# ishine/zerovox.cpp

Hardware: AMD Instinct MI355X
Metric: audio-seconds/wall-second (xRT) end-to-end phoneme->22.05 kHz wav (higher is better)
Workload: dtype f16*f16->f32 (MFMA) convs, f32 (MFMA) attention/linear, f32 activations

## Files before the change

zerovox.cpp_amd/csrc/capi.cpp:

```cpp
#include <algorithm>
#include <cmath>
#include <cstring>
#include <map>
#include <optional>
#include <string>
#include <thread>
#include <vector>

#include "common.h"
#include "model.h"
#include "knobs.h"

using zv::Model;

struct PendingBatch;
struct zv_model
{
    Model        *m;
    PendingBatch *pending;
};

static void free_pending(zv_model *m);
static void lane0_select(zv_model *m);
static void use_lane0(zv_model *m);
// ... 287 lines not shown
        const size_t b_ctl = r.prosody || tg ? zv::CTL_STRIDE * 4 : 0, b_pctl = pc ? (size_t)n * zv::PCTL_STRIDE * 4 : 0;
        if (!taps) M.reserve(n, T);
        Layout L;
        const size_t o_nf = L.at(4), o_ids = L.at(b_ids), o_pun = L.at(b_ids), o_sty = L.at(E * 4), o_ctl = L.at(b_ctl),
                     o_pctl = L.at(b_pctl), o_hid = L.at(b_hid);
        const size_t o_mel = taps ? 0 : L.at((size_t)T * M.hp.audio_num_mels * 4), o_wav = taps ? 0 : L.at(b_wav),
                     o_cum = taps ? 0 : L.at(dur ? b_ids : 0), o_live = L.at(r.fitted && !taps ? sizeof(zv::Seg) : 0),
                     o_runs = L.at(!r.fitted && !taps ? sizeof(zv::Seg) : 0);
        char *io = (char *)M.io_scratch(L.size());
        int32_t *d_nf = (int32_t *)(io + o_nf), *d_ids = (int32_t *)(io + o_ids), *d_pun = (int32_t *)(io + o_pun);
        float *d_sty = (float *)(io + o_sty), *d_hid = (float *)(io + o_hid);
        std::vector<float> ctl(b_ctl / 4), pctl(b_pctl / 4);
        std::vector<int32_t> cum(dur ? n : 0);
        pack_controls(r, ctl.data(), pctl.data());
        zv::Batch bt = zv::Batch::single(n, T, r.num_phonemes[0]);
        bt.has_targets = tg;
        if (r.fitted && !taps) bt.d_frm_live = (zv::Seg *)(io + o_live);
        if (!taps && M.dec_runs_on(bt)) bt.d_dec_runs = (zv::Seg *)(io + o_runs);
        ZV_HIP(hipMemcpyAsync(d_ids, r.ids[0], b_ids, hipMemcpyHostToDevice, M.stream()));
        ZV_HIP(hipMemcpyAsync(d_pun, r.puncts[0], b_ids, hipMemcpyHostToDevice, M.stream()));
        ZV_HIP(hipMemcpyAsync(d_sty, r.styles[0], E * 4, hipMemcpyHostToDevice, M.stream()));
        if (b_ctl)
        {
            bt.d_ctl = (const float *)(io + o_ctl);
            ZV_HIP(hipMemcpyAsync(io + o_ctl, ctl.data(), b_ctl, hipMemcpyHostToDevice, M.stream()));
        }
        if (b_pctl)
        {
            bt.d_pctl = (const float *)(io + o_pctl);
            ZV_HIP(hipMemcpyAsync(io + o_pctl, pctl.data(), b_pctl, hipMemcpyHostToDevice, M.stream()));
        }
        int32_t nf = 0;
        if (taps)
        {
            const Model::EncoderTaps t = M.encode_dev(bt, d_ids, d_pun, d_sty, d_hid, d_nf);
            ZV_HIP(hipMemcpyAsync(r.out[0], d_hid, b_hid, hipMemcpyDeviceToHost, M.stream()));
            ZV_HIP(hipMemcpyAsync(&nf, d_nf, 4, hipMemcpyDeviceToHost, M.stream()));
            if (taps->features) ZV_HIP(hipMemcpyAsync(taps->features, t.features, (size_t)n * E * 4, hipMemcpyDeviceToHost, M.stream()));
            if (taps->logdur) ZV_HIP(hipMemcpyAsync(taps->logdur, t.logdur, b_ids, hipMemcpyDeviceToHost, M.stream()));
            if (taps->pitch) ZV_HIP(hipMemcpyAsync(taps->pitch, t.pitch, b_ids, hipMemcpyDeviceToHost, M.stream()));
            if (taps->energy) ZV_HIP(hipMemcpyAsync(taps->energy, t.energy, b_ids, hipMemcpyDeviceToHost, M.stream()));
            if (taps->pitch_bucket) ZV_HIP(hipMemcpyAsync(taps->pitch_bucket, t.pitch_bucket, b_ids, hipMemcpyDeviceToHost, M.stream()));
            if (taps->energy_bucket) ZV_HIP(hipMemcpyAsync(taps->energy_bucket, t.energy_bucket, b_ids, hipMemcpyDeviceToHost, M.stream()));
            if (dur) ZV_HIP(hipMemcpyAsync(cum.data(), t.cum, b_ids, hipMemcpyDeviceToHost, M.stream()));
        }
        else
        {
            float *d_mel = (float *)(io + o_mel), *d_wav = (float *)(io + o_wav);
            if (dur) bt.d_cum = (int32_t *)(io + o_cum);
            M.chain_dev(bt, d_ids, d_pun, d_sty, d_hid, d_mel, d_wav, d_nf);
            ZV_HIP(hipMemcpyAsync(&nf, d_nf, 4, hipMemcpyDeviceToHost, M.stream()));
            if (dur) ZV_HIP(hipMemcpyAsync(cum.data(), bt.d_cum, b_ids, hipMemcpyDeviceToHost, M.stream()));
            ZV_HIP(hipMemcpyAsync(r.out[0], d_wav, b_wav, hipMemcpyDeviceToHost, M.stream()));
        }
        M.sync();
        if (r.n_frames) r.n_frames[0] = (uint32_t)nf;
        if (dur) durations_from_cum(cum.data(), 1, r.n, r.T, r.durations);
    });
}

zv_status zv_encode_taps(zv_model *m, const int32_t *ids, const int32_t *puncts, const float *style, uint32_t n,
                         uint32_t num_phonemes, uint32_t T, float *hidden, uint32_t *n_frames, float *features, float *logdur,
                         float *pitch, float *energy, int32_t *pitch_bucket, int32_t *energy_bucket)
{
    return run_single(m, {__func__, 1, &ids, &puncts, &style, &n, &num_phonemes, &T, &hidden, n_frames},
                      Taps{features, logdur, pitch, energy, pitch_bucket, energy_bucket});
}

zv_status zv_encode_taps_prosody(zv_model *m, const int32_t *ids, const int32_t *puncts, const float *style, uint32_t n,
                                 uint32_t num_phonemes, uint32_t T, float *hidden, uint32_t *n_frames, float *features, float *logdur,
                                 float *pitch, float *energy, int32_t *pitch_bucket, int32_t *energy_bucket, const zv_prosody *prosody)
{
    return run_single(m, {__func__, 1, &ids, &puncts, &style, &n, &num_phonemes, &T, &hidden, n_frames, prosody},
                      Taps{features, logdur, pitch, energy, pitch_bucket, energy_bucket});
}

zv_status zv_encode_taps_phonemes(zv_model *m, const int32_t *ids, const int32_t *puncts, const float *style, uint32_t n,
                                  uint32_t num_phonemes, uint32_t T, float *hidden, uint32_t *n_frames, float *features, float *logdur,
                                  float *pitch, float *energy, int32_t *pitch_bucket, int32_t *energy_bucket, const zv_prosody *prosody,
                                  const zv_phoneme_controls *phonemes, int32_t *durations)
{
    return run_single(m, {__func__, 1, &ids, &puncts, &style, &n, &num_phonemes, &T, &hidden, n_frames, prosody, phonemes, &durations},
                      Taps{features, logdur, pitch, energy, pitch_bucket, energy_bucket});
}

zv_status zv_encode(zv_model *m, const int32_t *ids, const int32_t *puncts, const float *style, uint32_t n, uint32_t T,
                    float *hidden, uint32_t *n_frames)
{
    return zv_encode_taps(m, ids, puncts, style, n, n, T, hidden, n_frames, nullptr, nullptr, nullptr, nullptr, nullptr, nullptr);
}

zv_status zv_decode(zv_model *m, const float *hidden, const float *style, uint32_t T, float *mel)
{
    return guarded([&] {
        ZV_NEED(m && hidden && style && mel, "null argument");
        Model &M = *m->m;
        use_lane0(m);
        check_T(M, T);
        const size_t E = M.E(), b_hid = (size_t)T * E * 4, b_mel = (size_t)T * M.hp.audio_num_mels * 4;
        Layout L;
        const size_t o_sty = L.at(E * 4), o_hid = L.at(b_hid), o_mel = L.at(b_mel);
        char *io = (char *)M.io_scratch(L.size());
        float *d_sty = (float *)(io + o_sty), *d_hid = (float *)(io + o_hid), *d_mel = (float *)(io + o_mel);
        ZV_HIP(hipMemcpyAsync(d_hid, hidden, b_hid, hipMemcpyHostToDevice, M.stream()));
        ZV_HIP(hipMemcpyAsync(d_sty, style, E * 4, hipMemcpyHostToDevice, M.stream()));
        M.decode_dev(zv::Batch::single(1, T, 1), d_hid, d_sty, d_mel);
        ZV_HIP(hipMemcpyAsync(mel, d_mel, b_mel, hipMemcpyDeviceToHost, M.stream()));
        M.sync();
    });
}

zv_status zv_vocode(zv_model *m, const float *mel, uint32_t T, float *wav)
{
    return guarded([&] {
        ZV_NEED(m && mel && wav, "null argument");
        Model &M = *m->m;
        use_lane0(m);
        check_T(M, T);
        const size_t b_mel = (size_t)T * M.hp.audio_num_mels * 4, b_wav = (size_t)T * M.hp.audio_hop_size * 4;
        Layout L;
        const size_t o_mel = L.at(b_mel), o_wav = L.at(b_wav);
        char *io = (char *)M.io_scratch(L.size());
        float *d_mel = (float *)(io + o_mel), *d_wav = (float *)(io + o_wav);
        ZV_HIP(hipMemcpyAsync(d_mel, mel, b_mel, hipMemcpyHostToDevice, M.stream()));
        M.vocode_dev_graph(zv::Batch::single(1, T, 1), d_mel, d_wav);
        ZV_HIP(hipMemcpyAsync(wav, d_wav, b_wav, hipMemcpyDeviceToHost, M.stream()));
        M.sync();
    });
}

uint32_t zv_vocoder_halo_frames(zv_model *m) { return m ? m->m->vocoder_halo_frames() : 0; }

zv_status zv_vocode_stream(zv_model *m, const float *mel, uint32_t T, uint32_t chunk_frames, zv_wav_sink sink, void *user)
{
    return guarded([&] {
        ZV_NEED(m && mel && sink, "null argument");
        ZV_NEED(T > 0 && chunk_frames > 0, "T and chunk_frames must be > 0");
        Model &M = *m->m;
        use_lane0(m);
        const size_t Mm = M.hp.audio_num_mels, hop = M.hp.audio_hop_size;
        const uint32_t H = M.vocoder_halo_frames();
        const uint32_t ctx_max = std::min<uint64_t>(T, (uint64_t)chunk_frames + 2 * H);
        check_T(M, ctx_max);
        struct RunsOff { Model &M; ~RunsOff() { M.voc_runs_off = false; } } runs_off{M};
        M.voc_runs_off = true;
        M.reserve(1, ctx_max);
        Layout L;
        const size_t o_mel = L.at((size_t)T * Mm * 4), o_wav = L.at((size_t)ctx_max * hop * 4);
        char *io = (char *)M.io_scratch(L.size());
        float *d_mel = (float *)(io + o_mel), *d_wav = (float *)(io + o_wav);
        Layout P;
        const size_t slot[2] = {P.at((size_t)chunk_frames * hop * 4), P.at((size_t)chunk_frames * hop * 4)};
        char *pin = (char *)M.pinned_scratch(P.size());
        hipEvent_t done[2] = {nullptr, nullptr};
        ZV_HIP(hipEventCreateWithFlags(&done[0], hipEventDisableTiming));
        ZV_HIP(hipEventCreateWithFlags(&done[1], hipEventDisableTiming));
        struct Pending { bool live; uint64_t first, n; } pend[2] = {{false, 0, 0}, {false, 0, 0}};
        auto deliver = [&](int k) {
            if (!pend[k].live) return;
            ZV_HIP(hipEventSynchronize(done[k]));
            sink(user, (const float *)(pin + slot[k]), pend[k].first, pend[k].n);
            pend[k].live = false;
        };
        try
        {
            ZV_HIP(hipMemcpyAsync(d_mel, mel, (size_t)T * Mm * 4, hipMemcpyHostToDevice, M.stream()));
            int k = 0;
            for (uint32_t a = 0; a < T; a += chunk_frames, k ^= 1)
            {
                const uint32_t b = std::min<uint64_t>(T, (uint64_t)a + chunk_frames);
                const uint32_t c0 = a > H ? a - H : 0, c1 = std::min<uint64_t>(T, (uint64_t)b + H);
                deliver(k);
                M.vocode_dev(zv::Batch::single(1, c1 - c0, 1), d_mel + (size_t)c0 * Mm, d_wav);
                ZV_HIP(hipMemcpyAsync(pin + slot[k], d_wav + (size_t)(a - c0) * hop, (size_t)(b - a) * hop * 4, hipMemcpyDeviceToHost, M.stream()));
                ZV_HIP(hipEventRecord(done[k], M.stream()));
                pend[k] = {true, (uint64_t)a * hop, (uint64_t)(b - a) * hop};
                deliver(k ^ 1);
            }
            deliver(k);
            deliver(k ^ 1);
        }
        catch (...)
        {
            hipStreamSynchronize(M.stream());
            hipEventDestroy(done[0]);
            hipEventDestroy(done[1]);
            throw;
        }
        M.sync();
        hipEventDestroy(done[0]);
        hipEventDestroy(done[1]);
    });
}

zv_status zv_synthesize(zv_model *m, const int32_t *ids, const int32_t *puncts, const float *style, uint32_t n, uint32_t T,
                        float *wav, uint32_t *n_frames)
{
    return run_single(m, {__func__, 1, &ids, &puncts, &style, &n, &n, &T, &wav, n_frames});
}

zv_status zv_synthesize_prosody(zv_model *m, const int32_t *ids, const int32_t *puncts, const float *style, uint32_t n, uint32_t T,
                                float *wav, uint32_t *n_frames, const zv_prosody *prosody)
{
    return run_single(m, {__func__, 1, &ids, &puncts, &style, &n, &n, &T, &wav, n_frames, prosody});
}

zv_status zv_synthesize_phonemes(zv_model *m, const int32_t *ids, const int32_t *puncts, const float *style, uint32_t n, uint32_t T,
                                 float *wav, uint32_t *n_frames, const zv_prosody *prosody, const zv_phoneme_controls *phonemes,
                                 int32_t *durations)
{
    return run_single(m, {__func__, 1, &ids, &puncts, &style, &n, &n, &T, &wav, n_frames, prosody, phonemes, &durations});
}

static void scatter_out(const char *pin_wav, const size_t *off, float *const *wav, const uint32_t *T, size_t hop, uint32_t a, uint32_t b)
{
    size_t total = 0;
    for (uint32_t u = a; u < b; u++) total += (size_t)T[u] * hop * 4;
    const unsigned nth = total > ((size_t)1 << 20) ? 4u : 1u;
    auto work = [&](unsigned k) {
        for (uint32_t u = a + k; u < b; u += nth) memcpy(wav[u], pin_wav + off[u], (size_t)T[u] * hop * 4);
    };
    if (nth == 1)
    {
        work(0);
        return;
    }
    std::vector<std::thread> th;
    for (unsigned k = 1; k < nth; k++) th.emplace_back(work, k);
    work(0);
    for (auto &t : th) t.join();
}

struct PendingBatch
{
    bool                  active = false;
    uint32_t              n_utt = 0;
    int                   G = 1;
    std::vector<uint32_t> gb;
    std::vector<size_t>   woff;
    std::vector<uint32_t> T;
    std::vector<float *>  wav;
    uint32_t             *n_frames = nullptr;
    const char           *h_wav = nullptr;
    const int32_t        *h_nf = nullptr;
    size_t                hop = 0;
    std::vector<uint32_t> N;
    std::vector<int32_t *> dur;
    const int32_t        *h_cum = nullptr;
};
static PendingBatch &pending_slot(zv_model *m, int lane)
{
    if (!m->pending) m->pending = new PendingBatch[ZV_BATCH_LANES];
    return m->pending[lane];
}
static void free_pending(zv_model *m)
{
    delete[] m->pending;
    m->pending = nullptr;
}
static void lane0_select(zv_model *m)
{
    if (hipSetDevice(m->m->device) != hipSuccess) zv::fail(ZV_ERR_DEVICE, "hipSetDevice(%d) failed", m->m->device);
    m->m->select_lane(0);
}
static void use_lane0(zv_model *m)
{
    if (m->pending && m->pending[0].active)
        zv::fail(ZV_ERR_ARG, "lane 0 has a batch in flight (zv_synthesize_batch_begin): finish it with zv_synthesize_batch_end first");
    if (hipSetDevice(m->m->device) != hipSuccess) zv::fail(ZV_ERR_DEVICE, "hipSetDevice(%d) failed", m->m->device);
    m->m->select_lane(0);
}

static void batch_enqueue(zv_model *m, int lane, const Request &r)
{
    Model &M = *m->m;
    PendingBatch &pb = pending_slot(m, lane);
    if (pb.active) zv::fail(ZV_ERR_ARG, "lane %d already has a batch in flight", lane);
    M.select_lane(lane);
    const size_t E = M.E(), Mm = M.hp.audio_num_mels, hop = M.hp.audio_hop_size;
    const bool tg = r.targets(), pc = r.phoneme_controls() || tg, ctl = r.prosody || tg, dur = r.timings();
    uint32_t nmax = 0, tmax = 0, ntot = 0;
    for (uint32_t u = 0; u < r.count; u++)
    {
        nmax = std::max(nmax, r.n[u]);
        tmax = std::max(tmax, r.T[u]);
        ntot += r.n[u];
    }
    zv::Batch bt;
    bt.nseg = (int)r.count;
    bt.n_max = zv::round_up((int)nmax, 32);
    bt.n_real = (int)nmax;
    bt.t_max = zv::round_up((int)tmax, 64);
    bt.n_rows = (size_t)bt.nseg * bt.n_max;
    bt.t_rows = (size_t)bt.nseg * bt.t_max;
    Layout in;
    const size_t b_tab = (size_t)(bt.nseg + 1) * sizeof(zv::Seg);
    const size_t i_tok = in.at(b_tab), i_frm = in.at(b_tab), i_ids = in.at(bt.n_rows * 4), i_pun = in.at(bt.n_rows * 4),
                 i_sty = in.at((size_t)bt.nseg * E * 4), i_ctl = in.at(ctl ? (size_t)bt.nseg * zv::CTL_STRIDE * 4 : 0),
                 i_pctl = in.at(pc ? bt.n_rows * zv::PCTL_STRIDE * 4 : 0), b_in = in.size();
    Layout dev;
    const size_t o_nf = dev.at((size_t)bt.nseg * 4), o_in = dev.at(b_in), o_hid = dev.at(bt.t_rows * E * 4),
                 o_mel = dev.at(bt.t_rows * Mm * 4), o_wav = dev.at(bt.t_rows * hop * 4), o_cum = dev.at(dur ? bt.n_rows * 4 : 0),
                 o_live = dev.at(r.fitted ? (size_t)bt.nseg * sizeof(zv::Seg) : 0),
                 o_runs = dev.at(!r.fitted ? (size_t)bt.nseg * sizeof(zv::Seg) : 0);
    M.reserve_batch(bt);
    char *io = (char *)M.io_scratch(dev.size());
    size_t wav_bytes = 0;
    pb.woff.assign(r.count, 0);
    for (uint32_t u = 0; u < r.count; u++)
    {
        pb.woff[u] = wav_bytes;
        wav_bytes += (size_t)r.T[u] * hop * 4;
    }
    Layout host;
    const size_t p_in = host.at(b_in), p_nf = host.at((size_t)bt.nseg * 4), p_wav = host.at(wav_bytes),
                 p_cum = host.at(dur ? bt.n_rows * 4 : 0);
    char *pin = (char *)M.pinned_scratch(host.size());
    char *d_in = io + o_in, *h_in = pin + p_in;
    {
        zv::Seg *h_tok = (zv::Seg *)(h_in + i_tok), *h_frm = (zv::Seg *)(h_in + i_frm);
        int32_t *h_ids = (int32_t *)(h_in + i_ids), *h_pun = (int32_t *)(h_in + i_pun);
        float *h_sty = (float *)(h_in + i_sty);
        int32_t n0 = 0, t0 = 0;
        for (uint32_t u = 0; u < r.count; u++)
        {
            const int32_t n = (int32_t)r.n[u], t = (int32_t)r.T[u];
            h_tok[u] = zv::Seg{n0, n, n, 0};
            h_frm[u] = zv::Seg{t0, t, 0, 0};
            memcpy(h_ids + n0, r.ids[u], (size_t)n * 4);
            memcpy(h_pun + n0, r.puncts[u], (size_t)n * 4);
            memcpy(h_sty + (size_t)u * E, r.styles[u], E * 4);
            n0 += n;
            t0 += t;
        }
        h_tok[r.count] = zv::Seg{0, n0, n0, 0};
        h_frm[r.count] = zv::Seg{0, t0, 0, 0};
        pack_controls(r, (float *)(h_in + i_ctl), (float *)(h_in + i_pctl));
    }
    bt.d_tok = (const zv::Seg *)(d_in + i_tok);
    bt.d_frm = (const zv::Seg *)(d_in + i_frm);
    if (ctl) bt.d_ctl = (const float *)(d_in + i_ctl);
    bt.has_targets = tg;
    if (pc) bt.d_pctl = (const float *)(d_in + i_pctl);
    if (dur) bt.d_cum = (int32_t *)(io + o_cum);
    if (r.fitted) bt.d_frm_live = (zv::Seg *)(io + o_live);
    if (M.dec_runs_on(bt)) bt.d_dec_runs = (zv::Seg *)(io + o_runs);
    int32_t *d_nf = (int32_t *)(io + o_nf), *d_ids = (int32_t *)(d_in + i_ids), *d_pun = (int32_t *)(d_in + i_pun);
    float *d_sty = (float *)(d_in + i_sty), *d_hid = (float *)(io + o_hid), *d_mel = (float *)(io + o_mel), *d_wav = (float *)(io + o_wav);
    int32_t *h_nf = (int32_t *)(pin + p_nf), *h_cum = dur ? (int32_t *)(pin + p_cum) : nullptr;
    char *h_wav = pin + p_wav;
    const int G = zv::voc_tail_groups(zv::knob(zv::ZV_TAIL_GROUPS), bt.nseg, wav_bytes, M.profiling, M.dbg_layer.kind >= 0);
    try
    {
        hipStream_t cs = M.copy_stream();
        pb.gb.assign(G + 1, r.count);
        pb.gb[0] = 0;
        const uint64_t seq = M.next_batch_seq();
        ZV_HIP(hipEventRecord(M.batch_event(seq, 0), M.stream()));
        if (G <= 1)
        {
            M.chain_dev(bt, d_ids, d_pun, d_sty, d_hid, d_mel, d_wav, d_nf, h_in, d_in, b_in);
            ZV_HIP(hipEventRecord(M.batch_event(seq, 1), M.stream()));
            ZV_HIP(hipMemcpyAsync(h_nf, d_nf, (size_t)bt.nseg * 4, hipMemcpyDeviceToHost, M.stream()));
            if (dur) ZV_HIP(hipMemcpyAsync(h_cum, bt.d_cum, (size_t)ntot * 4, hipMemcpyDeviceToHost, M.stream()));
            ZV_HIP(hipMemcpyAsync(h_wav, d_wav, wav_bytes, hipMemcpyDeviceToHost, M.stream()));
            ZV_HIP(hipEventRecord(M.tail_event(1), M.stream()));
        }
        else
        {
            M.chain_dev(bt, d_ids, d_pun, d_sty, d_hid, d_mel, d_wav, d_nf, h_in, d_in, b_in, 1);
            ZV_HIP(hipMemcpyAsync(h_nf, d_nf, (size_t)bt.nseg * 4, hipMemcpyDeviceToHost, M.stream()));
            if (dur) ZV_HIP(hipMemcpyAsync(h_cum, bt.d_cum, (size_t)ntot * 4, hipMemcpyDeviceToHost, M.stream()));
            for (int g = 1; g < G; g++)
            {
                uint32_t u = pb.gb[g - 1] + 1;
                while (u < r.count && pb.woff[u] < wav_bytes * g / G) u++;
                pb.gb[g] = std::min(u, r.count - (uint32_t)(G - g));
            }
            for (int g = 0; g < G; g++)
            {
                const uint32_t u0 = pb.gb[g], u1 = pb.gb[g + 1];
                M.vocode_tail(bt, d_mel, d_wav, (int)u0, (int)(u1 - u0));
                const size_t o0 = pb.woff[u0], o1 = u1 < r.count ? pb.woff[u1] : wav_bytes;
                ZV_HIP(hipEventRecord(M.tail_event(2 * g), M.stream()));
                ZV_HIP(hipStreamWaitEvent(cs, M.tail_event(2 * g), 0));
                ZV_HIP(hipMemcpyAsync(h_wav + o0, (const char *)d_wav + o0, o1 - o0, hipMemcpyDeviceToHost, cs));
                ZV_HIP(hipEventRecord(M.tail_event(2 * g + 1), cs));
            }
            ZV_HIP(hipEventRecord(M.batch_event(seq, 1), M.stream()));
        }
    }
    catch (...)
    {
        hipStreamSynchronize(M.stream());
        if (M.copy_stream()) hipStreamSynchronize(M.copy_stream());
        throw;
    }
    pb.active = true;
    pb.n_utt = r.count;
    pb.G = G;
    pb.T.assign(r.T, r.T + r.count);
    pb.wav.assign(r.out, r.out + r.count);
    pb.n_frames = r.n_frames;
    pb.h_wav = h_wav;
    pb.h_nf = h_nf;
    pb.hop = hop;
    pb.h_cum = h_cum;
    pb.N.assign(r.n, r.n + r.count);
    if (dur) pb.dur.assign(r.durations, r.durations + r.count);
    else pb.dur.clear();
}

static void batch_finish(zv_model *m, int lane)
{
    Model &M = *m->m;
    PendingBatch &pb = pending_slot(m, lane);
    if (!pb.active) zv::fail(ZV_ERR_ARG, "lane %d has no batch in flight", lane);
    M.select_lane(lane);
    try
    {
        for (int g = 0; g < pb.G; g++)
        {
            ZV_HIP(hipEventSynchronize(M.tail_event(2 * g + 1)));
            scatter_out(pb.h_wav, pb.woff.data(), pb.wav.data(), pb.T.data(), pb.hop, pb.gb[g], pb.gb[g + 1]);
        }
        M.sync();
    }
    catch (...)
    {
        hipStreamSynchronize(M.stream());
        if (M.copy_stream()) hipStreamSynchronize(M.copy_stream());
        pb.active = false;
        throw;
    }
    pb.active = false;
    if (pb.n_frames)
        for (uint32_t u = 0; u < pb.n_utt; u++) pb.n_frames[u] = (uint32_t)pb.h_nf[u];
    if (pb.h_cum) durations_from_cum(pb.h_cum, pb.n_utt, pb.N.data(), pb.T.data(), pb.dur.data());
}

static uint32_t batch_group_end(uint32_t a, uint32_t n_utt, const uint32_t *T)
{
    uint32_t b = a, tmax = 0;
    while (b < n_utt && b - a < 64)
    {
        const uint32_t tm = std::max(tmax, T[b]);
        if (b > a && (uint64_t)(b - a + 1) * zv::round_up((int)tm, 64) > 65536) break;
        tmax = tm;
        b++;
    }
    return b;
}

static zv_status synthesize_batch(zv_model *m, const Request &r)
{
      return guarded([&] {
        check_request(m, r);
        ZV_HIP(hipSetDevice(m->m->device));
        for (uint32_t a = 0, b; a < r.count; a = b)
        {
            b = batch_group_end(a, r.count, r.T);
            batch_enqueue(m, 0, r.slice(a, b));
            batch_finish(m, 0);
        }
    });
}

static zv_status begin_batch(zv_model *m, uint32_t lane, const Request &r)
{
    return guarded([&] {
        check_request(m, r);
        if (!(lane < ZV_BATCH_LANES)) zv::fail(ZV_ERR_ARG, "%s: lane out of range", r.fn);
        if (!(r.count > 0)) zv::fail(ZV_ERR_ARG, "%s: empty batch", r.fn);
        if (batch_group_end(0, r.count, r.T) != r.count)
            zv::fail(ZV_ERR_ARG, "%s: an asynchronous batch must fit one launch group (64 utterances, 64 Ki frames of capacity)", r.fn);
        ZV_HIP(hipSetDevice(m->m->device));
        batch_enqueue(m, (int)lane, r);
    });
}

zv_status zv_synthesize_batch(zv_model *m, uint32_t n_utt, const int32_t *const *ids, const int32_t *const *puncts,
                              const float *const *styles, const uint32_t *n_phonemes, const uint32_t *T, float *const *wav,
                              uint32_t *n_frames)
{
    return synthesize_batch(m, {__func__, n_utt, ids, puncts, styles, n_phonemes, n_phonemes, T, wav, n_frames});
}

zv_status zv_synthesize_batch_prosody(zv_model *m, uint32_t n_utt, const int32_t *const *ids, const int32_t *const *puncts,
                                      const float *const *styles, const uint32_t *n_phonemes, const uint32_t *T, float *const *wav,
                                      uint32_t *n_frames, const zv_prosody *prosody)
{
    return synthesize_batch(m, {__func__, n_utt, ids, puncts, styles, n_phonemes, n_phonemes, T, wav, n_frames, prosody});
}

zv_status zv_synthesize_batch_phonemes(zv_model *m, uint32_t n_utt, const int32_t *const *ids, const int32_t *const *puncts,
                                       const float *const *styles, const uint32_t *n_phonemes, const uint32_t *T, float *const *wav,
                                       uint32_t *n_frames, const zv_prosody *prosody, const zv_phoneme_controls *phonemes,
                                       int32_t *const *durations)
{
    return synthesize_batch(m, {__func__, n_utt, ids, puncts, styles, n_phonemes, n_phonemes, T, wav, n_frames, prosody, phonemes,
                                durations});
}

zv_status zv_synthesize_batch_begin(zv_model *m, uint32_t lane, uint32_t n_utt, const int32_t *const *ids, const int32_t *const *puncts,
                                    const float *const *styles, const uint32_t *n_phonemes, const uint32_t *T, float *const *wav,
                                    uint32_t *n_frames)
{
    return begin_batch(m, lane, {__func__, n_utt, ids, puncts, styles, n_phonemes, n_phonemes, T, wav, n_frames});
}

zv_status zv_synthesize_batch_begin_prosody(zv_model *m, uint32_t lane, uint32_t n_utt, const int32_t *const *ids,
                                            const int32_t *const *puncts, const float *const *styles, const uint32_t *n_phonemes,
                                            const uint32_t *T, float *const *wav, uint32_t *n_frames, const zv_prosody *prosody)
{
    return begin_batch(m, lane, {__func__, n_utt, ids, puncts, styles, n_phonemes, n_phonemes, T, wav, n_frames, prosody});
}

zv_status zv_synthesize_batch_begin_phonemes(zv_model *m, uint32_t lane, uint32_t n_utt, const int32_t *const *ids,
                                             const int32_t *const *puncts, const float *const *styles, const uint32_t *n_phonemes,
                                             const uint32_t *T, float *const *wav, uint32_t *n_frames, const zv_prosody *prosody,
                                             const zv_phoneme_controls *phonemes, int32_t *const *durations)
{
    return begin_batch(m, lane, {__func__, n_utt, ids, puncts, styles, n_phonemes, n_phonemes, T, wav, n_frames, prosody, phonemes,
                                 durations});
}

zv_status zv_synthesize_fitted(zv_model *m, const int32_t *ids, const int32_t *puncts, const float *style, uint32_t n, uint32_t T,
                               float *wav, uint32_t *n_frames, const zv_prosody *prosody, const zv_phoneme_controls *phonemes,
                               int32_t *durations)
{
    return run_single(m, {__func__, 1, &ids, &puncts, &style, &n, &n, &T, &wav, n_frames, prosody, phonemes, &durations, true});
}

zv_status zv_synthesize_batch_fitted(zv_model *m, uint32_t n_utt, const int32_t *const *ids, const int32_t *const *puncts,
                                     const float *const *styles, const uint32_t *n_phonemes, const uint32_t *T, float *const *wav,
                                     uint32_t *n_frames, const zv_prosody *prosody, const zv_phoneme_controls *phonemes,
                                     int32_t *const *durations)
{
    return synthesize_batch(m, {__func__, n_utt, ids, puncts, styles, n_phonemes, n_phonemes, T, wav, n_frames, prosody, phonemes,
                                durations, true});
}

zv_status zv_synthesize_batch_begin_fitted(zv_model *m, uint32_t lane, uint32_t n_utt, const int32_t *const *ids,
                                           const int32_t *const *puncts, const float *const *styles, const uint32_t *n_phonemes,
                                           const uint32_t *T, float *const *wav, uint32_t *n_frames, const zv_prosody *prosody,
                                           const zv_phoneme_controls *phonemes, int32_t *const *durations)
{
    return begin_batch(m, lane, {__func__, n_utt, ids, puncts, styles, n_phonemes, n_phonemes, T, wav, n_frames, prosody, phonemes,
                                 durations, true});
}

zv_status zv_encode_taps_target(zv_model *m, const int32_t *ids, const int32_t *puncts, const float *style, uint32_t n,
                                uint32_t num_phonemes, uint32_t T, float *hidden, uint32_t *n_frames, float *features, float *logdur,
                                float *pitch, float *energy, int32_t *pitch_bucket, int32_t *energy_bucket, const zv_prosody *prosody,
                                const zv_phoneme_controls *phonemes, int32_t *durations, uint32_t target_frames)
{
    return run_single(m, {__func__, 1, &ids, &puncts, &style, &n, &num_phonemes, &T, &hidden, n_frames, prosody, phonemes, &durations,
                          false, &target_frames},
                      Taps{features, logdur, pitch, energy, pitch_bucket, energy_bucket});
}

zv_status zv_synthesize_target(zv_model *m, const int32_t *ids, const int32_t *puncts, const float *style, uint32_t n, uint32_t T,
                               float *wav, uint32_t *n_frames, const zv_prosody *prosody, const zv_phoneme_controls *phonemes,
                               int32_t *durations, uint32_t target_frames, int fitted)
{
    return run_single(m, {__func__, 1, &ids, &puncts, &style, &n, &n, &T, &wav, n_frames, prosody, phonemes, &durations, fitted != 0,
                          &target_frames});
}

zv_status zv_synthesize_batch_target(zv_model *m, uint32_t n_utt, const int32_t *const *ids, const int32_t *const *puncts,
                                     const float *const *styles, const uint32_t *n_phonemes, const uint32_t *T, float *const *wav,
                                     uint32_t *n_frames, const zv_prosody *prosody, const zv_phoneme_controls *phonemes,
                                     int32_t *const *durations, const uint32_t *target_frames, int fitted)
{
    return synthesize_batch(m, {__func__, n_utt, ids, puncts, styles, n_phonemes, n_phonemes, T, wav, n_frames, prosody, phonemes,
                                durations, fitted != 0, target_frames});
}

zv_status zv_synthesize_batch_begin_target(zv_model *m, uint32_t lane, uint32_t n_utt, const int32_t *const *ids,
                                           const int32_t *const *puncts, const float *const *styles, const uint32_t *n_phonemes,
                                           const uint32_t *T, float *const *wav, uint32_t *n_frames, const zv_prosody *prosody,
                                           const zv_phoneme_controls *phonemes, int32_t *const *durations,
                                           const uint32_t *target_frames, int fitted)
{
    return begin_batch(m, lane, {__func__, n_utt, ids, puncts, styles, n_phonemes, n_phonemes, T, wav, n_frames, prosody, phonemes,
                                 durations, fitted != 0, target_frames});
}

zv_status zv_synthesize_batch_end(zv_model *m, uint32_t lane)
{
    return guarded([&] {
        ZV_NEED(m, "null argument");
        ZV_NEED(lane < ZV_BATCH_LANES, "lane out of range");
        ZV_HIP(hipSetDevice(m->m->device));
        batch_finish(m, (int)lane);
    });
}

zv_status zv_batch_timeline(zv_model *m, uint32_t cap, double *start_ms, double *end_ms, uint32_t *n)
{
    return guarded([&] {
        ZV_NEED(m && start_ms && end_ms && n, "null argument");
        Model &M = *m->m;
        ZV_HIP(hipSetDevice(M.device));
        M.sync_all_lanes();
        const uint64_t total = M.batch_seq();
        const uint64_t cnt = std::min<uint64_t>(std::min<uint64_t>(cap, total), (uint64_t)Model::BATCH_RING);
// ... 358 lines not shown
```

zerovox.cpp_amd/csrc/conv_plan.h:

```cpp
#pragma once

#include <stddef.h>

#include "conv_xcd.h"
#include "knobs.h"
#include "tile_deal.h"

namespace zv
{

constexpr long BATCH_ROWS = 16384;
inline bool batch_switch(int value, bool picked_by_itself) { return value != 0 && (value == 2 || picked_by_itself); }
inline bool batch_rows(long rows) { return rows >= BATCH_ROWS; }

constexpr size_t LDS_PER_WG = 160 * 1024;
constexpr size_t LDS_TWO_WGS = 80 * 1024;
constexpr size_t LDS_DEFAULT = 64 * 1024;

inline int plan_round_up(int x, int a) { return (x + a - 1) / a * a; }

struct ConvCall
{
    int njobs, nseg, max_rows, rate, n_cu, nt_begin;
};

inline int conv_gemm_groups(int Cout_p) { return ((Cout_p + 31) / 32) / 8; }
inline int conv_gemm_tiles(int Cout_p)
{
    const int nt = (Cout_p + 31) / 32, ng = nt / 8;
    return ng * 8 + ((nt - ng * 8 == 1 && ng >= 1) ? 1 : 0);
}
inline int conv_gemm_units(int Cin_p, int K)
{
    int n = 0;
    for (int c0 = 0; c0 < Cin_p; c0 += 256) n += K * (((Cin_p - c0 < 256 ? Cin_p - c0 : 256) + 63) / 64);
    return n;
}

enum ConvPrologue : int
{
    PRO_RAW_F16 = 0,
    PRO_ACT = 1,
    PRO_NORM_ACT = 2,
    PRO_MELNORM = 3,
    PRO_SUM3_ACT = 4,
    PRO_SCALE_ACT = 5
};

#ifndef ZV_SINGLE_LW
#define ZV_SINGLE_LW 4
#endif
#ifndef ZV_CONV_BATCH_ROUTE
#define ZV_CONV_BATCH_ROUTE 1
#endif

struct ConvDesc
{
    int  K, dil, pad, Cin_p, Cout_p, ck, pro, ldx;
    bool has_w8, out_f16, has_res, has_stat, eact, three_inputs;
};

inline bool conv_gemm_takes(const ConvDesc &j, const ConvCall &c)
{
    const long rows = (long)c.max_rows * c.rate * c.nseg;
    return batch_switch(knob(ZV_CONV_GEMM), batch_rows(rows)) && j.has_w8 && j.pro == PRO_RAW_F16 && j.Cin_p >= 128 &&
           conv_gemm_groups(j.Cout_p) >= 1 && !j.out_f16 && (j.ldx & 7) == 0;
}

struct ConvGemmPlan
{
    int    order, tps, gx, threads;
    size_t lds_bytes;
};
inline ConvGemmPlan conv_gemm_plan(int Cout_p, const ConvCall &c)
{
    ConvGemmPlan p{};
    p.order = knob(ZV_GEMM_ORDER);
    p.tps = (c.max_rows * c.rate + 255) / 256;
    const int ng = conv_gemm_groups(Cout_p), rts = p.tps * c.nseg;
    p.gx = (p.order == 1 && (ng == 1 || ng == 2 || ng == 4)) ? plan_round_up(rts, 8 / ng) * ng : rts * ng;
    p.threads = 512;
    p.lds_bytes = 4 * (16384 + 18432);
    return p;
}

inline bool conv_stream_ok(const ConvDesc &j, const ConvCall &c)
{
    return c.njobs == 1 && c.nt_begin == 0 && (j.pro == PRO_ACT || j.pro == PRO_SCALE_ACT) && j.K == 3 && j.dil == 1 && j.pad == 1 &&
           (j.Cin_p == 64 || j.Cin_p == 128) && j.ck == j.Cin_p && (j.ldx & 3) == 0 && !j.has_res && !j.has_stat && !j.eact && !j.out_f16 &&
           !j.three_inputs;
}

inline bool conv_tiled_exists(int MT, int WN, int NT)
{
    return (NT == 1 && (MT == 1 || MT == 2 || MT == 4) && (WN == 1 || WN == 2 || WN == 4)) || (NT == 2 && MT == 2 && WN == 4);
}

enum ConvForm { CONV_STREAM, CONV_LOADER, CONV_TILED };
struct ConvPlan
{
    bool     valid;
    ConvForm form;
    int      MT, WN, NT;
    int      strip, nkc;
    int      tps;
    int      gx, gy, gz, threads;
    size_t   lds_bytes;
    int      tile_bytes;
    int      xcd_nx, xcd_ny, xcd_spread;
    int      warm;
};

inline bool conv_plan_tiles(ConvPlan &p, bool loader, int MT, int WN, int NT, int Lmax, int ntiles, int halo, int ck, int dmax, const ConvCall &c)
{
    const int BM = 32 * MT * (4 / WN);
    p.form = loader ? CONV_LOADER : CONV_TILED;
    p.MT = MT, p.WN = WN, p.NT = NT;
    p.tps = (Lmax + BM - 1) / BM;
    p.gx = p.tps * c.nseg, p.gy = (ntiles + WN * NT - 1) / (WN * NT), p.gz = c.njobs;
    const int LW = loader ? ZV_SINGLE_LW : 0;
    p.threads = 256 + 64 * LW;
    p.xcd_nx = p.xcd_ny = p.xcd_spread = 0;
    p.warm = knob(ZV_CONV_WARM) != 0;
    if (loader && knob(ZV_CONV_XCD) != 0)
    {
        p.xcd_ny = p.gy;
        p.xcd_nx = p.gx;
        p.xcd_spread = c.nseg > 1;
        p.gx = conv_xcd_grid(p.xcd_nx, p.xcd_ny, p.xcd_spread), p.gy = 1;
    }
    p.tile_bytes = plan_round_up((BM + halo + dmax) * (ck * 2 + 16), 16);
    p.lds_bytes = (size_t)p.tile_bytes * (LW > 0 ? 2 : 1);
    return p.lds_bytes <= LDS_PER_WG;
}

inline ConvPlan conv_stream_plan(const ConvDesc &j, const ConvCall &c)
{
    ConvPlan p{};
    const int Lmax = c.max_rows * c.rate;
    const int ntiles = (j.Cout_p + 31) / 32, gy = (ntiles + 3) / 4;
    const int occ = j.Cin_p == 128 ? 2 : 3;
    int strip = 8;
    while (strip > 2 && (long)((Lmax + 64 * strip - 1) / (64 * strip)) * c.nseg * gy < 12L * occ * c.n_cu) strip >>= 1;
    p.valid = true;
    p.form = CONV_STREAM;
    p.strip = strip;
    p.nkc = j.Cin_p / 16;
    p.tps = (Lmax + 64 * strip - 1) / (64 * strip);
    p.gx = p.tps * c.nseg, p.gy = gy, p.gz = 1;
    p.threads = 256;
    p.lds_bytes = (size_t)2 * 66 * (j.Cin_p * 2 + 16);
    return p;
}

inline ConvPlan conv_plan(const ConvDesc *jobs, const ConvCall &c)
{
    ConvPlan p{};
    const int njobs = c.njobs, n_cu = c.n_cu;
    const int Lmax = c.max_rows * c.rate;
    if (njobs < 1) return p;
    int halo = 0, ck = 0, dmax = 1;
    for (int i = 0; i < njobs; i++)
    {
        dmax = jobs[i].dil > dmax ? jobs[i].dil : dmax;
        if (jobs[i].Cout_p != jobs[0].Cout_p) return p;
        const int h = (jobs[i].K - 1) * jobs[i].dil;
        if (h > halo) halo = h;
        ck = jobs[i].ck > ck ? jobs[i].ck : ck;
    }
    const int Cout_p = jobs[0].Cout_p;
    const int ntiles = (Cout_p + 31) / 32 - c.nt_begin;
    if (ntiles < 1) return p;
    const int WN = ntiles >= 3 ? 4 : (ntiles >= 2 ? 2 : 1);
    auto wgs = [&](int MT, int NT) {
        const int BM = 32 * MT * (4 / WN);
        return (long)((Lmax + BM - 1) / BM) * c.nseg * ((ntiles + WN * NT - 1) / (WN * NT)) * njobs;
    };
    int MT = 4;
    while (MT > 1 && wgs(MT, 1) < 2L * n_cu) MT >>= 1;
    while (MT > 1 && (size_t)(32 * MT * (4 / WN) + halo + dmax) * (ck * 2 + 16) > LDS_TWO_WGS) MT >>= 1;
    {
        const double ai = 2.0 * jobs[0].K * jobs[0].Cin_p * Cout_p / (4.0 * (jobs[0].Cin_p + Cout_p));
        const bool memory_bound = ai < 200.0 && wgs(1, 1) >= 16L * n_cu;
        if (conv_stream_ok(jobs[0], c) && batch_switch(knob(ZV_CONV_STREAM), memory_bound)) return conv_stream_plan(jobs[0], c);
        if (memory_bound && MT > 2) MT = 2;
    }
    if (MT < knob(ZV_CONV_MT)) MT = knob(ZV_CONV_MT);
    const int nt_env = knob(ZV_CONV_NT);
    int NT = (WN == 4 && ntiles >= 8 && MT >= 2 && wgs(MT, 2) >= 4L * n_cu && jobs[0].K * jobs[0].Cin_p >= 2048) ? 2 : 1;
    if (nt_env == 1 || (nt_env == 2 && WN == 4 && ntiles >= 2 && MT >= 2)) NT = nt_env;
    if (NT == 2 && MT == 4) MT = 2;
    {
        const bool batch_rounds = ZV_CONV_BATCH_ROUTE && c.nseg > 1 && wgs(1, 1) > n_cu;
        const int  single_env = knob(ZV_CONV_SINGLE);
        if (single_env != 0 && MT == 1 && NT == 1 && ck == 256 && wgs(1, 1) <= 2L * n_cu && !batch_rounds && (jobs[0].Cin_p > 256 || single_env == 2) &&
            WN >= 2 && conv_plan_tiles(p, true, 1, WN, 1, Lmax, ntiles, halo, ck, dmax, c))
        {
            p.valid = true;
            return p;
        }
    }
    p.valid = conv_tiled_exists(MT, WN, NT) && conv_plan_tiles(p, false, MT, WN, NT, Lmax, ntiles, halo, ck, dmax, c);
    return p;
}

constexpr int TRIPLE_MAX_DIL = 3;

struct BlockTile
{
    int sumd, dmax;
    int h2;
    int halo;
    int TM;
};
inline BlockTile block_tile(int K, const int *dil, int n_dil, int R)
{
    BlockTile t{0, 1, (K - 1) / 2, 0, 0};
    for (int d = 0; d < n_dil; d++)
    {
        t.sumd += dil[d];
        t.dmax = dil[d] > t.dmax ? dil[d] : t.dmax;
    }
    t.halo = t.h2 * (t.sumd + n_dil);
    t.TM = R - 2 * t.halo;
    return t;
}

struct BlockDesc
{
    int Cp, K, n_dil;
    int dil[TRIPLE_MAX_DIL];
};

inline bool pair_supported(int Cp, int K)
{
    if (!(Cp == 32 || Cp == 64 || Cp == 128 || Cp == 256) || K < 1 || (K & 1) == 0) return false;
    const int nsb = (K * (Cp / 16) + 3) >> 2;
    return nsb >= 2 && (Cp == 64 || (nsb & 1) == 0);
}
inline bool triple_supported(int Cp, int K, const int *dil, int n_dil)
{
    if (Cp != 32 || n_dil < 1 || n_dil > TRIPLE_MAX_DIL || !pair_supported(Cp, K) || (K & 1) == 0) return false;
    return block_tile(K, dil, n_dil, 256).TM >= 96;
}
inline bool block64_supported(int Cp, int K, const int *dil, int n_dil)
{
    if (Cp != 64 || K < 3 || (K & 1) == 0 || n_dil < 1 || n_dil > TRIPLE_MAX_DIL) return false;
    return block_tile(K, dil, n_dil, 256).TM >= 192;
}

struct PairPlan
{
    bool   valid;
    bool   ring;
    int    MT;
    int    deal_c, gx, gz;
    int    ring_off;
    size_t lds_bytes;
};
inline PairPlan pair_plan(int Cp, int Kmax, int dmax, bool any_sum, bool merged, bool all_ring_weights, const ConvCall &c)
{
    PairPlan p{};
    if (!(Cp == 32 || Cp == 64 || Cp == 128 || Cp == 256) || (any_sum && merged)) return p;
    const int  njobs = c.njobs, n_cu = c.n_cu, Lmax = c.max_rows * c.rate;
    const int  WN = Cp == 256 ? 4 : Cp / 32;
    auto wgs = [&](int MT) {
        const int BM = 32 * MT * (4 / WN);
        const int TM = BM - (Kmax - 1);
        return TM < 32 ? 0L : (long)((Lmax + TM - 1) / TM) * c.nseg * njobs;
    };
    p.deal_c = tile_deal_chunk(Cp);
    p.gz = merged ? 1 : njobs;
    {
        const int  ring_env = knob(ZV_PAIR64_RING);
        const bool ok = Cp == 64 && !any_sum && ring_env != 0 && Kmax >= 3 &&
                        (size_t)(256 + Kmax * dmax) * 144 + 4 * 8192 + 1024 <= LDS_TWO_WGS && all_ring_weights;
        const long rwgs = (long)((Lmax + 256 - Kmax) / (257 - Kmax)) * c.nseg * njobs;
        if (ok && (ring_env == 2 || rwgs >= 6L * n_cu))
        {
            const int BM = 256, TMmin = BM - (Kmax - 1);
            p.ring = true;
            p.gx = tile_deal_grid((Lmax + TMmin - 1) / TMmin, c.nseg, p.deal_c);
            p.ring_off = plan_round_up((BM + Kmax * dmax) * (64 * 2 + 16), 1024);
            p.lds_bytes = (size_t)p.ring_off + 4 * 8192;
            p.valid = p.lds_bytes <= LDS_TWO_WGS;
            return p;
        }
    }
    int MT = (Cp == 128 && wgs(4) >= 8L * n_cu) ? 4 : 2;
    if (Cp == 256 && !merged && wgs(3) >= 4L * n_cu) MT = 3;
    const int mt_env = knob(ZV_PAIR_MT);
    if (mt_env == 2 || mt_env == 4 || (mt_env == 3 && Cp == 256 && !merged)) MT = mt_env;
    p.MT = MT;
    const int BM = 32 * MT * (4 / WN);
    const int TMmin = BM - (Kmax - 1);
    if (TMmin < 32) return p;
    p.gx = tile_deal_grid((Lmax + TMmin - 1) / TMmin, c.nseg, p.deal_c);
    p.lds_bytes = (size_t)(BM + (Kmax + (Cp == 256 ? 0 : (Cp >= 128 ? 1 : 4))) * dmax) * (Cp * 2 + 16);
    p.valid = true;
    return p;
}

struct TriplePlan
{
    bool   valid;
    int    R, MT;
    bool   lds_form;
    int    db_mask;
    int    interleave;
    int    deal_c, gx, gz, threads;
    size_t lds_bytes;
};
inline TriplePlan triple_plan(const BlockDesc *jobs, const ConvCall &c)
{
    TriplePlan p{};
    const int njobs = c.njobs, Lmax = c.max_rows * c.rate;
    const int v2_env = knob(ZV_TRIPLE_V2);
    const int R = ((long)Lmax * c.nseg * njobs >= 7000L * c.n_cu || v2_env == 3) ? 512 : 256;
    p.R = R, p.MT = 2;
    p.deal_c = tile_deal_chunk(32);
    p.interleave = 1;
    int    gx = 8;
    size_t lds = 0, lds2 = 0;
    for (int i = 0; i < njobs; i++)
    {
        const BlockDesc &P = jobs[i];
        if (P.Cp != jobs[0].Cp || !triple_supported(P.Cp, P.K, P.dil, P.n_dil)) return p;
        const BlockTile t = block_tile(P.K, P.dil, P.n_dil, R);
        const int g = tile_deal_grid((Lmax + t.TM - 1) / t.TM, c.nseg, p.deal_c);
        gx = g > gx ? g : gx;
        const size_t rows = R + 2 * t.h2 * t.dmax + 5 * t.dmax;
        const size_t b = rows * (P.Cp * 2 + 16);
        lds = b > lds ? b : lds;
        const int    nb = ((P.K * 2 + 3) >> 2) >> 1;
        const size_t one = (size_t)plan_round_up((int)(rows * 80), 1024) + (size_t)(8 * nb + 2) * 1024 + 1024;
        const bool   db = knob(ZV_TRIPLE_DB) != 0 && one + (size_t)8 * nb * 1024 <= LDS_TWO_WGS;
        if (db) p.db_mask |= 1 << i;
        const size_t b2 = one + (db ? (size_t)8 * nb * 1024 : 0);
        lds2 = b2 > lds2 ? b2 : lds2;
    }
    if (njobs < 1 || lds > LDS_DEFAULT) return p;
    p.gx = gx, p.gz = njobs;
    if (v2_env && (R == 512 || v2_env >= 2) && lds2 <= LDS_TWO_WGS)
    {
        p.lds_form = true;
        p.interleave = knob(ZV_TRIPLE_INTERLEAVE) != 0 ? njobs : 1;
        if (p.interleave > 1) p.gx = gx * njobs, p.gz = 1;
        p.threads = R;
        p.lds_bytes = lds2;
        p.valid = true;
        return p;
    }
    p.db_mask = 0;
    p.threads = 64 * (R / 32 / p.MT);
    p.lds_bytes = lds;
    p.valid = true;
    return p;
}

struct Block64Plan
{
    bool   valid;
    int    deal_c, gx, gz, threads;
    int    ring_off;
    size_t lds_bytes;
};
inline Block64Plan block64_plan(const BlockDesc *jobs, const ConvCall &c)
{
    Block64Plan p{};
    const int Lmax = c.max_rows * c.rate;
    p.deal_c = tile_deal_chunk(64);
    int gx = 8, rows_max = 0;
    for (int i = 0; i < c.njobs; i++)
    {
        const BlockDesc &P = jobs[i];
        if (!block64_supported(P.Cp, P.K, P.dil, P.n_dil)) return p;
        const BlockTile t = block_tile(P.K, P.dil, P.n_dil, 256);
        const int g = tile_deal_grid((Lmax + t.TM - 1) / t.TM, c.nseg, p.deal_c);
        gx = g > gx ? g : gx;
        const int rows = 256 + 2 * t.h2 * t.dmax + 2 * t.dmax;
        rows_max = rows > rows_max ? rows : rows_max;
    }
    p.gx = gx, p.gz = c.njobs, p.threads = 256;
    p.ring_off = plan_round_up(rows_max * (64 * 2 + 16), 1024);
    p.lds_bytes = (size_t)p.ring_off + 4 * 8192;
    p.valid = c.njobs >= 1 && p.lds_bytes <= LDS_TWO_WGS;
    return p;
}

}
```

zerovox.cpp_amd/csrc/dec_runs.h:

```cpp
#pragma once

#include <stddef.h>

#if defined(__HIPCC__)
#define ZV_DR_FN __host__ __device__ static inline
#else
#define ZV_DR_FN static inline
#endif

namespace zv
{

constexpr int DEC_RUN_BLOCK = 32;
constexpr int DEC_RUN_MARGIN = 32;

struct DecRun
{
    int rows_c;
    int gap_at;
    int G;
};

ZV_DR_FN DecRun dec_run(int n, int T, int R)
{
    const DecRun whole = {T, 0, 0};
    n = n < 0 ? 0 : (n < T ? n : T);
    if (R < 0 || T - R - 1 < 0) return whole;
    const long a = ((long)n + R + 2 * DEC_RUN_BLOCK - 1) / DEC_RUN_BLOCK * DEC_RUN_BLOCK;
    const long b = (long)(T - R - 1) / DEC_RUN_BLOCK * DEC_RUN_BLOCK;
    if (b - a < DEC_RUN_BLOCK || b - a < DEC_RUN_MARGIN) return whole;
    const DecRun r = {(int)(a + (T - b)), (int)(a / DEC_RUN_BLOCK), (int)((b - a) / DEC_RUN_BLOCK)};
    return r;
}

ZV_DR_FN int dec_run_compact_row(int t, int gap_at, int G)
{
    const int a = gap_at * DEC_RUN_BLOCK, b = a + G * DEC_RUN_BLOCK;
    return (G <= 0 || t < a) ? t : (t < b ? a - 1 : t - G * DEC_RUN_BLOCK);
}
ZV_DR_FN int dec_run_original_row(int c, int gap_at, int G) { return (G <= 0 || c < gap_at * DEC_RUN_BLOCK) ? c : c + G * DEC_RUN_BLOCK; }

ZV_DR_FN void dec_run_block_sum(const double *p, size_t stride, int nb, int gap_at, int G, double *sum, double *sumsq)
{
    double s1 = 0.0, s2 = 0.0;
    for (int b0 = 0; b0 < nb; b0 += 8)
    {
        double v1[8], v2[8];
#if defined(__HIPCC__)
#pragma unroll
#endif
        for (int i = 0; i < 8; i++)
        {
            const double *q = p + (size_t)(b0 + i < nb ? b0 + i : nb - 1) * stride;
            v1[i] = q[0];
            v2[i] = q[1];
        }
#if defined(__HIPCC__)
#pragma unroll
#endif
        for (int i = 0; i < 8; i++)
            if (b0 + i < nb)
            {
                s1 += v1[i];
                s2 += v2[i];
                if (b0 + i + 1 == gap_at)
                    for (int k = 0; k < G; k++)
                    {
                        s1 += v1[i];
                        s2 += v2[i];
                    }
            }
    }
    *sum = s1;
    *sumsq = s2;
}

}
```

zerovox.cpp_amd/csrc/decoder.cpp:

```cpp
#include "schedule.h"

#include <algorithm>
#include <cmath>

namespace zv
{

Model::DecLayout Model::dec_layout(DeviceArena &a, const Batch &bt) const
{
    const size_t S = (size_t)bt.nseg, L = bt.t_rows, B = 2 * E(), R = (size_t)dec_.R, CAT = B + R;
    DecLayout d{(bt.t_max + 31) / 32, round_up(dec_.fc_out + 64, 64), 2 * (int)CAT + 64};
    d.h = a.take_n<float>(S * d.hs);
    for (float **st : {&d.st_x, &d.st_t, &d.st_y, &d.st_a}) *st = a.take_n<float>(S * d.ss);
    for (double **p : {&d.part_t, &d.part_o}) *p = a.take_n<double>(S * d.nblk * CAT * 2);
    d.cat = a.take_n<float>(L * CAT);
    for (float **x : {&d.t1, &d.sc, &d.x0, &d.xa}) *x = a.take_n<float>(L * B);
    d.asr_t = a.take_n<float>(L * R);
    d.xa16 = a.take_n<_Float16>(L * CAT);
    d.t16 = a.take_n<_Float16>(L * B);
    d.xr16 = a.take_n<_Float16>(L * CAT);
    d.mel_c = a.take_n<float>(L * dec_.M);
    return d;
}

bool Model::dec_prepass_on(const Batch &bt) const
{
    const int pre_env = knob(ZV_DEC_PREPASS);
    return pre_env >= 0 ? pre_env != 0 : (size_t)bt.t_max * bt.nseg >= 256;
}

bool Model::dec_runs_on(const Batch &bt) const
{
    const int k = knob(ZV_DEC_RUNS);
    return !bt.d_frm_live && dbg_layer.kind < 0 && dec_prepass_on(bt) && batch_switch(k, batch_rows((long)bt.t_rows));
}

int Model::dec_reach_frames() const
{
    auto half = [](const ConvW &w) { return w.K > 0 ? (w.K - 1) / 2 : 0; };
    auto blk = [&](const DecBlk &b) { return std::max(half(b.conv1) + half(b.conv2), b.learned_sc ? half(b.sc) : 0); };
    int r = std::max(blk(dec_.enc[0]) + blk(dec_.enc[1]), half(dec_.asr0));
    for (const DecBlk &b : dec_.dec) r += blk(b);
    return r + half(dec_.to_out);
}

void Model::decode_dev(const Batch &bt, const float *d_hidden, const float *d_styles, float *d_mel)
{
    if (bt.t_rows == 0 || bt.t_max <= 0) fail(ZV_ERR_ARG, "T must be > 0");
    const DecLayout lay = dec_layout(stage_arena(bt), bt);
    const bool runs = bt.d_dec_runs != nullptr;
    if (runs && !dec_runs_on(bt)) fail(ZV_ERR_ARG, "internal: a decoder run table on a schedule that takes none");
    const Segs fr = runs ? Segs{bt.d_dec_runs, bt.nseg, bt.t_max, bt.frm1} : bt.frames();
    const int Ed = (int)E(), B = 2 * Ed, R = dec_.R, CAT = B + R, S = bt.nseg;
    const size_t L = bt.t_rows;
    const int nblk = lay.nblk, hs = lay.hs, ss = lay.ss;
    float *const h = lay.h, *const st_x = lay.st_x, *const st_t = lay.st_t, *const st_y = lay.st_y, *const st_a = lay.st_a;
    double *const part_t = lay.part_t, *const part_o = lay.part_o;
    float *const cat = lay.cat, *const t1 = lay.t1, *const sc = lay.sc, *const x0 = lay.x0, *const xa = lay.xa, *const asr_t = lay.asr_t;
    _Float16 *const xa16 = lay.xa16, *const t16 = lay.t16, *const xr16 = lay.xr16;
    double Ld = (double)L;
    if (runs && profiling)
    {
        std::vector<Seg> tab((size_t)S);
        ZV_HIP(hipMemcpyAsync(tab.data(), bt.d_dec_runs, tab.size() * sizeof(Seg), hipMemcpyDeviceToHost, stream()));
        ZV_HIP(hipStreamSynchronize(stream()));
        Ld = 0;
        for (const Seg &g : tab) Ld += g.rows;
    }
    const bool prepass = dec_prepass_on(bt);

    ZV_LAUNCH("dec_adain_fc", 4.0 * dec_.fc_out * (Ed + 2), 2.0 * S * dec_.fc_out * Ed,
              launch_linear(stream(), d_styles, Ed, Ed, dec_.fcW, dec_.fcB, dec_.fc_out, h, hs, dec_.fcExtra, segs_single(S)));

    const float rsqrt2 = (float)(1.0 / sqrt(2.0));

    auto finalize = [&](const double *part, int C, float *stat, int c_off) {
        ZV_LAUNCH("dec_in_stats", 16.0 * S * nblk * C, 4.0 * S * nblk * C,
                  launch_stats_finalize(stream(), part, nblk, C, 1e-5f, stat, ss, c_off, fr, 1, runs));
    };
    auto norm_input = [&](ConvJob &j, const float *x, int ldx, int C, const double *part, int Cpart, float *stat, const float *g,
                          const float *b, int gb_seg, _Float16 *op16, _Float16 *raw16 = nullptr) {
        if (prepass)
        {
            ZV_LAUNCH("dec_norm_operand", 6.0 * Ld * C, 8.0 * Ld * C,
                      launch_norm_act_f16(stream(), x, ldx, C, part, nblk, Cpart, 1e-5f, stat, ss, g, b, gb_seg, 0.2f, op16, C, fr, raw16, runs));
            j.x0 = op16;
            j.ldx = C;
            j.pro = PRO_RAW_F16;
        }
        else
        {
            finalize(part, Cpart, stat, 0);
            j.x0 = x;
            j.ldx = ldx;
            j.pro = PRO_NORM_ACT;
            j.pstat = stat;
            j.pstat_seg = ss;
            j.pa = g;
            j.pb = b;
            j.pab_seg = gb_seg;
            j.slope = 0.2f;
        }
    };

    ZV_LAUNCH("dec_in_stats", 4.0 * Ld * Ed, 3.0 * Ld * Ed, launch_stats_partial(stream(), d_hidden, Ed, Ed, part_o, nblk, fr, 1));

    int blk_no = 0;
    auto block = [&](const DecBlk &b, const float *x, int ldx, int Cpart, float *st_in, const float *g1, const float *b1,
                     const float *g2, const float *b2, int gb_seg, float *out, int ldo, bool want_stats) {
        const bool dbg_here = dbg_layer.kind == 2 && dbg_layer.index == blk_no && !dbg_layer.done;
        blk_no++;
        if (dbg_layer.done) return;
        if (dbg_here)
        {
            dbg_inject(const_cast<float *>(x), ldx, b.cin, L);
            ZV_HIP(launch_stats_partial(stream(), x, ldx, b.cin, part_o, nblk, fr, 1));
            Cpart = b.cin;
        }
        const float *res = x;
        int ldres = ldx;
        ConvJob jj[2];
        int nj = 0;
        {
            ConvJob j = job(b.conv1);
            norm_input(j, x, ldx, b.cin, part_o, Cpart, st_in, g1, b1, gb_seg, xa16, b.learned_sc ? xr16 : nullptr);
            j.out = t1;
            j.stat_part = part_t;
            j.stat_nblk = nblk;
            j.stat_C = b.conv1.Cout;
            jj[nj++] = j;
        }
        double bytes = conv_bytes(Ld, b.cin, b.conv1.Cout, 3, false), flops = conv_flops(Ld, b.cin, b.conv1.Cout, 3);
        if (b.learned_sc)
        {
            ConvJob j = job(b.sc);
            j.x0 = x;
            j.ldx = ldx;
            if (prepass)
            {
                j.x0 = xr16;
                j.ldx = b.cin;
                j.pro = PRO_RAW_F16;
            }
            j.out = sc;
            res = sc;
            ldres = b.sc.Cout_p;
            const double sb = conv_bytes(Ld, b.cin, b.cout, 1, false), sf = conv_flops(Ld, b.cin, b.cout, 1);
            if (b.sc.Cout_p == b.conv1.Cout_p)
            {
                jj[nj++] = j;
                bytes += sb;
                flops += sf;
            }
            else
                conv(&j, 1, fr, 1, "dec_conv", sb, sf);
        }
        conv(jj, nj, fr, 1, "dec_conv", bytes, flops);
        const int Cm = b.conv1.Cout;
        {
            ConvJob j = job(b.conv2);
            norm_input(j, t1, b.conv1.Cout_p, Cm, part_t, Cm, st_t, g2, b2, gb_seg, t16);
            j.res = res;
            j.ldres = ldres;
            j.escale = rsqrt2;
            j.out = out;
            j.ldo = ldo;
            if (want_stats)
            {
                j.stat_part = part_o;
                j.stat_nblk = nblk;
                j.stat_C = b.cout;
            }
            conv(&j, 1, fr, 1, "dec_conv", conv_bytes(Ld, Cm, b.cout, 3, true), conv_flops(Ld, Cm, b.cout, 3));
        }
        if (dbg_here) dbg_extract(out, ldo, b.cout, L);
    };

    if (dbg_layer.kind == ZV_LAYER_DEC_ADAIN)
    {
        const int bi = dbg_layer.index / 2, k = dbg_layer.index & 1;
        if (bi < 0 || bi >= 5) return;
        const DecBlk &b = dec_.dec[bi];
        const int Cn = k ? b.cout : b.cin, go = k ? b.g2 : b.g1;
        float *xin = cat;
        dbg_inject(xin, Cn, Cn, L);
        ZV_HIP(launch_stats_partial(stream(), xin, Cn, Cn, part_o, nblk, fr, 1));
        ZV_HIP(launch_stats_finalize(stream(), part_o, nblk, Cn, 1e-5f, st_x, ss, 0, fr, 1));
        ZV_HIP(launch_norm_apply(stream(), xin, Cn, Cn, st_x, ss, h + go, h + go + Cn, t1, Cn, nullptr, nblk, fr));
        dbg_extract(t1, Cn, Cn, L);
        return;
    }

    block(dec_.enc[0], d_hidden, Ed, Ed, st_x, dec_.enc[0].n1w, dec_.enc[0].n1b, dec_.enc[0].n2w, dec_.enc[0].n2b, 0, x0, B, true);
    block(dec_.enc[1], x0, B, B, st_y, dec_.enc[1].n1w, dec_.enc[1].n1b, dec_.enc[1].n2w, dec_.enc[1].n2b, 0, cat, CAT, true);

    if (dbg_layer.done) return;
    {
        ConvJob j = job(dec_.asr0);
        j.x0 = d_hidden;
        j.ldx = Ed;
        j.out = asr_t;
        j.stat_part = part_t;
        j.stat_nblk = nblk;
        j.stat_C = R;
        conv(&j, 1, fr, 1, "dec_conv", conv_bytes(Ld, Ed, R, 1, false), conv_flops(Ld, Ed, R, 1));
        finalize(part_t, R, st_a, 0);
        ZV_LAUNCH("dec_norm_apply", 8.0 * Ld * R, 3.0 * Ld * R,
                  launch_norm_apply(stream(), asr_t, R, R, st_a, ss, dec_.asr1w, dec_.asr1b, cat + B, CAT, part_t, nblk, fr));
        finalize(part_t, R, st_x, B);
        if (dbg_layer.kind == ZV_LAYER_DEC_ASR_RES)
        {
            dbg_extract(cat + B, CAT, R, L);
            return;
        }
    }

    const float *cur = cat;
    int ldc = CAT;
    float *outs[5] = {cat, cat, xa, x0, xa};
    const int ldos[5] = {CAT, CAT, Ed, Ed, Ed};
    const int cparts[5] = {B, B, B, Ed, Ed};
    float *sts[5] = {st_x, st_x, st_x, st_y, st_y};
    for (int i = 0; i < 5; i++)
    {
        const DecBlk &b = dec_.dec[i];
        block(b, cur, ldc, cparts[i], sts[i], h + b.g1, h + b.g1 + b.cin, h + b.g2, h + b.g2 + b.cout, hs, outs[i], ldos[i], i < 4);
        cur = outs[i];
        ldc = ldos[i];
    }
    if (dbg_layer.done) return;
    {
        ConvJob j = job(dec_.to_out);
        j.x0 = cur;
        j.ldx = ldc;
        j.out = runs ? lay.mel_c : d_mel;
        j.ldo = dec_.M;
        if (dbg_layer.kind == ZV_LAYER_DEC_TO_OUT) dbg_inject(const_cast<float *>(cur), ldc, Ed, L);
        conv(&j, 1, fr, 1, "dec_conv", conv_bytes(Ld, Ed, dec_.M, 1, false), conv_flops(Ld, Ed, dec_.M, 1));
        if (dbg_layer.kind == ZV_LAYER_DEC_TO_OUT) dbg_extract(d_mel, dec_.M, dec_.M, L);
    }
    if (runs)
        ZV_LAUNCH("dec_run_expand", 4.0 * (Ld + (double)L) * dec_.M, 0.0,
                  launch_dec_run_expand(stream(), lay.mel_c, d_mel, dec_.M, fr, bt.frames_cap()));
}

}
```

zerovox.cpp_amd/csrc/encoder.cpp:

```cpp
#include "schedule.h"

#include <cmath>

namespace zv
{

Model::EncLayout Model::enc_layout(DeviceArena &a, const Batch &bt) const
{
    const size_t n = bt.n_rows, Ed = E();
    EncLayout e{round_up(enc_.dur.V, 16)};
    for (float **p : {&e.x, &e.y}) *p = a.take_n<float>(n * Ed);
    e.qkv = a.take_n<float>(n * 3 * Ed);
    for (float **p : {&e.o, &e.f}) *p = a.take_n<float>(n * Ed);
    e.hh = a.take_n<_Float16>(n * round_up(hp.conv_filter_size, 16));
    for (float **p : {&e.va, &e.vb}) *p = a.take_n<float>(n * e.Vp);
    for (float **p : {&e.t.logdur, &e.t.pitch, &e.t.energy}) *p = a.take_n<float>(n);
    for (int32_t **p : {&e.t.pitch_bucket, &e.t.energy_bucket}) *p = a.take_n<int32_t>(n);
    e.t.cum = bt.d_cum ? bt.d_cum : a.take_n<int32_t>(n);
    e.t.features = e.x;
    return e;
}

Model::EncoderTaps Model::encode_dev(const Batch &bt, const int32_t *d_ids, const int32_t *d_puncts, const float *d_styles,
                                     float *d_hidden, int32_t *d_nframes)
{
    if (bt.n_rows == 0 || bt.t_rows == 0 || bt.n_max <= 0 || bt.t_max <= 0) fail(ZV_ERR_ARG, "N and T must be > 0");
    const int n_longest = bt.n_real > 0 ? bt.n_real : bt.n_max;
    if (n_longest > enc_.posenc_rows) fail(ZV_ERR_ARG, "%d phonemes exceed the %d rows of the sinusoid table", n_longest, enc_.posenc_rows);
    const EncLayout lay = enc_layout(stage_arena(bt), bt);
    const Segs tk = bt.tokens(), fr = bt.frames_cap();
    const Segs tkm = knob(ZV_LINEAR_MERGED) != 0 ? bt.tokens_merged() : tk;
    const int Ed = (int)E(), H = hp.encoder_head, dk = Ed / H;
    const size_t n = bt.n_rows;
    const double nd = (double)n;
    const int Vp = lay.Vp;
    float *const x = lay.x, *const y = lay.y, *const qkv = lay.qkv, *const o = lay.o, *const f = lay.f, *const va = lay.va, *const vb = lay.vb;
    _Float16 *const hh = lay.hh;
    const bool tails = dbg_layer.kind < 0 && knob(ZV_LN_TAIL) != 0 && layernorm_tail_ok(Ed) && layernorm_tail_ok(enc_.dur.V);
    const EncoderTaps t = lay.t;

    ZV_LAUNCH("enc_embed", 8.0 * nd * Ed, 1.0 * nd * Ed,
              launch_embed(stream(), d_ids, d_puncts, enc_.wemb, hp.emb_dim, enc_.pemb, hp.punct_emb_dim, enc_.posenc, x, Ed, tk));
    if (dbg_layer.kind == ZV_LAYER_ENC_EMBED)
    {
        dbg_extract(x, Ed, Ed, n);
        return t;
    }
    const float temperature = (float)pow((double)dk, 0.5);
    const float inv_t = (float)(1.0 / temperature);
    int layer_no = 0;
    for (const EncLayer &Ly : enc_.layers)
    {
        const bool dbg_here = dbg_layer.kind == 1 && dbg_layer.index == layer_no;
        const bool dbg_mha = dbg_layer.kind == ZV_LAYER_ENC_MHA && dbg_layer.index == layer_no;
        const bool dbg_ffn = dbg_layer.kind == ZV_LAYER_ENC_FFN && dbg_layer.index == layer_no;
        layer_no++;
        if (dbg_here || dbg_mha) dbg_inject(x, Ed, Ed, n);
        ZV_LAUNCH("enc_linear", 4.0 * (3.0 * Ed * Ed + 4.0 * nd * Ed), 6.0 * nd * Ed * Ed,
                  launch_linear(stream(), x, Ed, Ed, Ly.qkvW, Ly.qkvB, 3 * Ed, qkv, 3 * Ed, nullptr, tkm));
        ZV_LAUNCH("enc_attention", 16.0 * nd * Ed, 4.0 * nd * bt.n_max * Ed,
                  launch_attention(stream(), qkv, qkv + Ed, qkv + 2 * Ed, 3 * Ed, H, dk, inv_t, o, Ed, tk));
        ZV_LAUNCH("enc_linear", 4.0 * (1.0 * Ed * Ed + 2.0 * nd * Ed), 2.0 * nd * Ed * Ed,
                  launch_linear(stream(), o, Ed, Ed, Ly.fcW, Ly.fcB, Ed, f, Ed, nullptr, tkm));
        ZV_LAUNCH("enc_layernorm", 12.0 * nd * Ed, 8.0 * nd * Ed,
                  launch_add_layernorm(stream(), f, Ed, x, Ed, Ed, Ed, Ly.ln1w, Ly.ln1b, 1e-5f, y, Ed, tkm));
        if (dbg_mha)
        {
            dbg_extract(y, Ed, Ed, n);
            return t;
        }
        if (dbg_ffn) dbg_inject(y, Ed, Ed, n);
        {
            ConvJob a = job(Ly.w1);
            a.x0 = y;
            a.eact = 1;
            a.oslope = 0.f;
            a.out_f16 = 1;
            a.out = hh;
            conv(&a, 1, tk, 1, "enc_conv", conv_bytes(nd, Ed, Ly.w1.Cout, Ly.w1.K, false), conv_flops(nd, Ed, Ly.w1.Cout, Ly.w1.K));
            ConvJob b = job(Ly.w2);
            b.x0 = hh;
            b.pro = PRO_RAW_F16;
            b.out = f;
            conv(&b, 1, Ly.w2.K == 1 ? tkm : tk, 1, "enc_conv", conv_bytes(nd, Ly.w1.Cout, Ed, Ly.w2.K, false), conv_flops(nd, Ly.w1.Cout, Ed, Ly.w2.K));
        }
        if (tails && layer_no == (int)enc_.layers.size())
            ZV_LAUNCH("enc_layernorm", 12.0 * nd * Ed, 9.0 * nd * Ed,
                      launch_layernorm_tail(stream(), f, Ed, y, Ed, Ed, Ed, Ly.ln2w, Ly.ln2b, 1e-5f, x, Ed, tk, d_styles, Ed, nullptr, nullptr,
                                            nullptr, nullptr, 0, 0, nullptr, 0, nullptr));
        else
            ZV_LAUNCH("enc_layernorm", 12.0 * nd * Ed, 8.0 * nd * Ed,
                      launch_add_layernorm(stream(), f, Ed, y, Ed, Ed, Ed, Ly.ln2w, Ly.ln2b, 1e-5f, x, Ed, tkm));
        if (dbg_here || dbg_ffn)
        {
            dbg_extract(x, Ed, Ed, n);
            return t;
        }
    }
    if (!(tails && !enc_.layers.empty()))
        ZV_LAUNCH("enc_add_style", 8.0 * nd * Ed, 1.0 * nd * Ed, launch_add_rowvec(stream(), x, Ed, Ed, d_styles, Ed, tk));

    int pred_no = 0;
    auto predictor = [&](const VarPred &v, float *out, const float *emb, int32_t *bucket, int ctl_field, int pctl_field) {
        const float *pctl = emb && bt.d_pctl ? bt.d_pctl + pctl_field : nullptr;
        const bool dbg_here = dbg_layer.kind == 3 && dbg_layer.index == pred_no && !dbg_layer.done;
        pred_no++;
        if (dbg_layer.done) return;
        if (dbg_here) dbg_inject(x, Ed, Ed, n);
        ConvJob a = job(v.c1);
        a.x0 = x;
        a.eact = 1;
        a.oslope = 0.f;
        a.out = va;
        conv(&a, 1, tk, 1, "enc_conv", conv_bytes(nd, Ed, v.V, 3, false), conv_flops(nd, Ed, v.V, 3));
        ZV_LAUNCH("enc_layernorm", 8.0 * nd * v.V, 8.0 * nd * v.V,
                  launch_add_layernorm(stream(), va, Vp, nullptr, 0, v.V, Vp, v.l1w, v.l1b, 1e-5f, vb, Vp, tkm));
        ConvJob b = job(v.c2);
        b.x0 = vb;
        b.pad = 1;
        b.eact = 1;
        b.oslope = 0.f;
        b.out = va;
        conv(&b, 1, tk, 1, "enc_conv", conv_bytes(nd, v.V, v.V, 3, false), conv_flops(nd, v.V, v.V, 3));
        if (tails)
        {
            ZV_LAUNCH("enc_layernorm", 8.0 * nd * v.V + (emb ? 12.0 * nd * Ed : 0.0), 10.0 * nd * v.V,
                      launch_layernorm_tail(stream(), va, Vp, nullptr, 0, v.V, Vp, v.l2w, v.l2b, 1e-5f, vb, Vp, tk, nullptr, 0, v.lw, v.lb, out,
                                            emb, (int)hp.encoder_ve_n_bins, Ed, x, Ed, bucket, emb ? bt.d_ctl : nullptr, ctl_field, pctl));
            return;
        }
        ZV_LAUNCH("enc_layernorm", 8.0 * nd * v.V, 8.0 * nd * v.V,
                  launch_add_layernorm(stream(), va, Vp, nullptr, 0, v.V, Vp, v.l2w, v.l2b, 1e-5f, vb, Vp, tkm));
        ZV_LAUNCH("enc_rowdot", 4.0 * nd * v.V, 2.0 * nd * v.V, launch_rowdot(stream(), vb, Vp, v.V, v.lw, v.lb, out, tk));
        if (dbg_here) dbg_extract(out, 1, 1, n);
        if (emb && !dbg_layer.done)
            ZV_LAUNCH("enc_bucket_embed", 12.0 * nd * Ed, 1.0 * nd * Ed,
                      launch_bucket_embed_add(stream(), out, hp.encoder_ve_n_bins, emb, Ed, x, Ed, bucket, tk, bt.d_ctl, ctl_field, pctl));
    };
    predictor(enc_.dur, t.logdur, nullptr, nullptr, 0, 0);
    predictor(enc_.pitch, t.pitch, enc_.pitch_emb, t.pitch_bucket, CTL_PITCH, PCTL_PITCH);
    if (dbg_layer.done) return t;
    predictor(enc_.energy, t.energy, enc_.energy_emb, t.energy_bucket, CTL_ENERGY, PCTL_ENERGY);
    if (dbg_layer.done) return t;
    if (bt.has_targets)
    {
        if (!bt.d_ctl || !bt.d_pctl) fail(ZV_ERR_ARG, "a batch with target durations needs its control rows");
        ZV_LAUNCH("enc_fit_durations", 24.0 * nd, 0.0, launch_fit_durations(stream(), t.logdur, bt.d_ctl, bt.d_pctl, tk, fr));
    }
    ZV_LAUNCH("enc_length_regulator", 4.0 * (nd + (double)bt.t_rows) * Ed, 0.0,
              launch_length_regulator(stream(), x, Ed, t.logdur, Ed, d_hidden, Ed, t.cum, d_nframes, tk, fr, bt.d_ctl, bt.d_pctl));
    if (bt.d_frm_live)
        ZV_LAUNCH("enc_live_frames", 36.0 * bt.nseg, 0.0, launch_live_frames(stream(), d_nframes, bt.d_frm_live, fr));
    if (bt.d_dec_runs)
        ZV_LAUNCH("enc_dec_runs", 36.0 * bt.nseg, 0.0, launch_dec_runs(stream(), d_nframes, bt.d_dec_runs, fr, dec_reach_frames()));
    return t;
}

void Model::debug_layernorm(int index, uint32_t n)
{
    const int l = index >> 1, Ed = (int)E();
    if (index < 0 || l >= (int)enc_.layers.size()) return;
    const EncLayer &Ly = enc_.layers[l];
    float *d = (float *)io_scratch(2 * (size_t)n * Ed * 4), *y = d + (size_t)n * Ed;
    dbg_inject(d, Ed, Ed, n);
    ZV_HIP(launch_add_layernorm(stream(), d, Ed, nullptr, 0, Ed, Ed, (index & 1) ? Ly.ln2w : Ly.ln1w, (index & 1) ? Ly.ln2b : Ly.ln1b,
                                1e-5f, y, Ed, segs_single((int)n)));
    dbg_extract(y, Ed, Ed, n);
}

}
```

zerovox.cpp_amd/csrc/kernels.h:

```cpp
#pragma once

#include <hip/hip_runtime.h>
#include <stdint.h>

#include "conv_plan.h"
#include "voc_plan.h"

#ifdef ZV_DIAG
#define ZV_DBGBITS(x) (x)
#else
#define ZV_DBGBITS(x) 0
#endif

namespace zv
{

__host__ __device__ static inline int round_up(int x, int a) { return (x + a - 1) / a * a; }

struct Seg
{
    int32_t row0, rows;
    int32_t aux;
    int32_t pad;
};
struct Segs
{
    const Seg *tab;
    int        nseg;
    int        max_rows;
    Seg        one;
};
__host__ __device__ static inline Seg seg_at(const Segs &s, int u)
{
    Seg g = s.tab ? s.tab[u] : s.one;
#if defined(__HIP_DEVICE_COMPILE__)
    g.row0 = __builtin_amdgcn_readfirstlane(g.row0);
    g.rows = __builtin_amdgcn_readfirstlane(g.rows);
    g.aux = __builtin_amdgcn_readfirstlane(g.aux);
#endif
    return g;
}
static inline Segs segs_single(int rows, int aux = 0)
{
    Segs s;
    s.tab = nullptr;
    s.nseg = 1;
    s.max_rows = rows;
    s.one.row0 = 0;
    s.one.rows = rows;
    s.one.aux = aux;
    s.one.pad = 0;
    return s;
}


struct ConvJob
{
    const void  *x0, *x1, *x2;
    int          ldx;
    int          pro;
    float        slope, pscale;
    const float *pa, *pb;
    const float *pstat;
    int          L, Cin_p, Cout_p, K, dil, pad;
    int          ck;
    const void  *w;
    const void  *w8;
    const float *bias;
    const float *res;
    int          ldres;
    float        escale;
    int          eact;
    float        oslope;
    int          out_f16;
    void        *out;
    int          ldo;
    int          dbg;
    int          pstat_seg, pab_seg;
    double      *stat_part;
    int          stat_nblk, stat_C;
};

constexpr int CONV_MAX_JOBS = 4;
struct ConvJobs
{
    ConvJob j[CONV_MAX_JOBS];
    Segs    segs;
    int     rate;
    int     tps;
    int     nt_begin;
    int     order;
    int     tile_bytes;
    int     xcd_ny, xcd_nx;
    int     xcd_spread;
    int     warm;
#ifdef ZV_STAMPS
    unsigned long long *stamp;
#endif
};

size_t packed_conv_weight_halfs(int Cin_p, int Cout_p, int K);
int    conv_pick_ck(int Cin_p, int ck_max = 0);
void   pack_conv_weight(const uint16_t *w, int K, int IC, int OC, int Cin_p, int Cout_p, int ck, uint16_t *dst);
size_t conv_gemm_weight_halfs(int Cin_p, int Cout_p, int K);
void   pack_conv_weight_gemm(const uint16_t *w, int K, int IC, int OC, int Cin_p, int Cout_p, uint16_t *dst);
hipError_t launch_conv(hipStream_t s, const ConvJob *jobs, int njobs, int n_cu, const Segs &segs, int rate);

struct PairJob
{
    const float *y;
    float       *out;
    const void  *w1, *w2;
    const void  *w1r, *w2r;
    const float *b1, *b2;
    int          L, Cp, K, dil;
    float        slope;
    int          dbg;
    const float *sum_in;
    float       *sum_out;
};
constexpr int PAIR_MAX_JOBS = 3;
struct PairJobs
{
    PairJob j[PAIR_MAX_JOBS];
    Segs    segs;
    int     rate;
    int     njobs, kmax;
    int     deal_c;
#ifdef ZV_STAMPS
    unsigned long long *stamp;
#endif
    float  *merge_out;
    int     ring_off;
};
size_t     pair_weight_halfs(int Cp, int K);
void       pack_pair_weight(const uint16_t *w, int K, int C, int Cp, uint16_t *dst);
size_t     pair_weight16_halfs(int Cp, int K);
void       pack_pair_weight16(const uint16_t *w, int K, int C, int Cp, uint16_t *dst, bool conv2_layout);
size_t     pair_ring_weight_halfs(int Cp, int K);
void       pack_pair_weight_ring(const uint16_t *w, int K, int C, int Cp, uint16_t *dst, bool conv2_layout);
hipError_t launch_pair(hipStream_t s, const PairJob *jobs, int njobs, int n_cu, const Segs &segs, int rate, float *merge_out = nullptr);

struct TripleJob
{
    const float *y;
    float       *out;
    const void  *w1[TRIPLE_MAX_DIL], *w2[TRIPLE_MAX_DIL];
    const void  *w1x[TRIPLE_MAX_DIL], *w2x[TRIPLE_MAX_DIL];
    const float *b1[TRIPLE_MAX_DIL], *b2[TRIPLE_MAX_DIL];
    int          dil[TRIPLE_MAX_DIL];
    int          n_dil;
    int          L, Cp, K;
    float        slope;
    int          dbg;
};
struct TripleJobs
{
    TripleJob j[PAIR_MAX_JOBS];
    Segs      segs;
    int       rate;
    int       deal_c;
    int       interleave;
    int       db_mask;
    int       ring_off;
#ifdef ZV_STAMPS
    unsigned long long *stamp;
#endif
};
hipError_t launch_block64(hipStream_t s, const TripleJob *jobs, int njobs, const Segs &segs, int rate);
hipError_t launch_triple(hipStream_t s, const TripleJob *jobs, int njobs, int n_cu, const Segs &segs, int rate);

struct OutConvArgs
{
    const float *x0, *x1, *x2;
    int          ldx, L, C, K;
    float        pscale, slope;
    const uint16_t *w;
    float        bias;
    float       *out;
    Segs         segs;
    int          rate;
    int          runs;
};
hipError_t launch_out_conv(hipStream_t s, const OutConvArgs &a);

hipError_t launch_stats_partial(hipStream_t s, const float *x, int ldx, int C, double *part, int nblk, const Segs &segs, int rate);
hipError_t launch_stats_finalize(hipStream_t s, const double *part, int nblk, int C, float eps, float *stat, int stat_seg,
                                 int c_off, const Segs &segs, int rate, int dec_runs = 0);
hipError_t launch_norm_apply(hipStream_t s, const float *x, int ldx, int C, const float *stat, int stat_seg, const float *g,
                             const float *b, float *y, int ldy, double *part, int nblk, const Segs &segs);

hipError_t launch_act_f16(hipStream_t s, const float *x0, const float *x1, const float *x2, float pscale, float slope, void *out, size_t n);
hipError_t launch_norm_act_f16(hipStream_t s, const float *x, int ldx, int C, const double *part, int nblk, int Cpart, float eps,
                               float *stat, int stat_seg, const float *ga, const float *be, int gb_seg, float slope, void *y,
                               int ldy, const Segs &segs, void *yraw = nullptr, int dec_runs = 0);

hipError_t launch_linear(hipStream_t s, const float *x, int ldx, int in, const float *W, const float *b, int out, float *y,
                         int ldy, const float *extra, const Segs &segs);

hipError_t launch_embed(hipStream_t s, const int32_t *ids, const int32_t *puncts, const float *wemb, int emb,
                        const float *pemb, int pdim, const float *posenc, float *x, int ld, const Segs &segs);
hipError_t launch_attention(hipStream_t s, const float *q, const float *k, const float *v, int ld, int H, int dk,
                            float inv_temp, float *o, int ldo, const Segs &segs);
constexpr int CTL_STRIDE = 8;
constexpr int CTL_DURATION = 0;
constexpr int CTL_PITCH = 1;
constexpr int CTL_ENERGY = 3;
constexpr int CTL_TARGET = 5;
constexpr int PCTL_STRIDE = 4;
constexpr int PCTL_FRAMES = 0;
constexpr int PCTL_DURATION = 1;
constexpr int PCTL_PITCH = 2;
constexpr int PCTL_ENERGY = 3;

hipError_t launch_add_layernorm(hipStream_t s, const float *x, int ldx, const float *res, int ldr, int C, int Cp,
                                const float *w, const float *b, float eps, float *y, int ldy, const Segs &segs);
bool       layernorm_tail_ok(int C);
hipError_t launch_layernorm_tail(hipStream_t s, const float *x, int ldx, const float *res, int ldr, int C, int Cp, const float *w,
                                 const float *b, float eps, float *y, int ldy, const Segs &segs, const float *post, int post_seg,
                                 const float *dot_w, const float *dot_b, float *pred, const float *emb, int nbins, int embC, float *feat,
                                 int ldf, int32_t *bucket, const float *ctl = nullptr, int ctl_field = 0,
                                 const float *pctl = nullptr);
hipError_t launch_add_rowvec(hipStream_t s, float *x, int ld, int C, const float *v, int v_seg, const Segs &segs);
hipError_t launch_rowdot(hipStream_t s, const float *x, int ld, int C, const float *w, const float *b, float *y, const Segs &segs);
hipError_t launch_bucket_embed_add(hipStream_t s, const float *pred, int nbins, const float *emb, int C, float *x, int ld,
                                   int32_t *bucket, const Segs &segs, const float *ctl = nullptr, int ctl_field = 0,
                                   const float *pctl = nullptr);
hipError_t launch_length_regulator(hipStream_t s, const float *feat, int ld, const float *logdur, int C, float *hidden,
                                   int ldh, int32_t *cum, int32_t *n_frames, const Segs &tokens, const Segs &frames,
                                   const float *ctl = nullptr, const float *pctl = nullptr);

constexpr int FIT_MAX_TOKENS = 3584;
hipError_t launch_fit_durations(hipStream_t s, const float *logdur, const float *ctl, const float *pctl, const Segs &tokens,
                                const Segs &frames);

hipError_t launch_live_frames(hipStream_t s, const int32_t *n_frames, Seg *live, const Segs &frames);
hipError_t launch_zero_tail(hipStream_t s, float *x, int C, const Segs &frames, const Segs &live, int rate);

constexpr int VOC_RUN_MARGIN = 16;
hipError_t launch_voc_runs(hipStream_t s, const float *mel, int M, float *mel_c, int32_t *eq, Seg *runs, const Segs &frames, int H);
hipError_t launch_voc_run_fill(hipStream_t s, float *x, const Segs &runs, int rate);

hipError_t launch_dec_runs(hipStream_t s, const int32_t *n_frames, Seg *runs, const Segs &frames, int R);
hipError_t launch_dec_run_expand(hipStream_t s, const float *mel_c, float *mel, int M, const Segs &runs, const Segs &frames);

}
```

zerovox.cpp_amd/csrc/knobs.h:

```cpp
#pragma once

namespace zv
{

#define ZV_KNOB_LIST(X)                                                                                                               \
    X(ZV_NO_FUSE, 0)                                                                  \
    X(ZV_NO_TRIPLE, 0)                                                                          \
    X(ZV_FUSE256, 0)                                                \
    X(ZV_NO_MERGE, 0)                                                               \
    X(ZV_MERGE_ALWAYS, 0)                 \
    X(ZV_MERGE_SEQ, 1)          \
    X(ZV_MERGE_MAXC, 256)                                  \
    X(ZV_TAIL_GROUPS, 8)                                                        \
    X(ZV_ARENA_FILL, 0)                                         \
    X(ZV_DEC_PREPASS, -1)                                      \
    X(ZV_CONV_MT, 0)                                                              \
    X(ZV_CONV_NT, 0)                                                     \
    X(ZV_CONV_SINGLE, 1)                                    \
    X(ZV_CONV_GEMM, 1)                  \
    X(ZV_CONV_STREAM, 1)        \
    X(ZV_VOC_RUNS, 1)           \
    X(ZV_DEC_RUNS, 1)           \
    X(ZV_UP_GEMM, 1)            \
    X(ZV_GEMM_ORDER, 2)         \
    X(ZV_PAIR_MT, 0)                                                                  \
    X(ZV_CONV_XCD, 1)           \
    X(ZV_CONV_WARM, 1)          \
    X(ZV_LINEAR_MERGED, 1)      \
    X(ZV_BLOCK64, 3)            \
    X(ZV_PAIR64_RING, 1)               \
    X(ZV_TRIPLE_V2, 1)                               \
    X(ZV_TRIPLE_DB, 1)                                                                     \
    X(ZV_TRIPLE_INTERLEAVE, 1)                                                               \
    X(ZV_ATT_SCALAR, 0)                                                                               \
    X(ZV_ATT_MFMA, 0)                                                          \
    X(ZV_LN_TAIL, 1)

#ifdef ZV_DIAG
#define ZV_KNOB_LIST_DIAG(X)                                                                                                          \
    X(ZV_DBG, 0)                                                                       \
    X(ZV_LDS_PAD, 0)            \
    X(ZV_STAMP_CP, 0)                               \
    X(ZV_STAMP_CONV, 0)                                    \
    X(ZV_STAMP_CIN, 0)
#else
#define ZV_KNOB_LIST_DIAG(X)
#endif

enum Knob : int
{
#define ZV_KNOB_ENUM(n, d) n,
    ZV_KNOB_LIST(ZV_KNOB_ENUM)
    ZV_KNOB_LIST_DIAG(ZV_KNOB_ENUM)
#undef ZV_KNOB_ENUM
    ZV_KNOB_COUNT
};

int         knob(Knob k);
bool        knob_set(const char *name, int value);
void        knob_reset();
bool        knob_get(const char *name, int *value);
unsigned    knob_epoch();
const char *knob_name(int k);
#ifdef ZV_DIAG
inline int diag_bits() { return knob(ZV_DBG); }
#else
inline int diag_bits() { return 0; }
#endif

}
```

zerovox.cpp_amd/csrc/misc_kernels.hip:

```cpp
#include "kernels.h"
#include "knobs.h"
#include "fit_durations.h"
#include "dec_runs.h"

#include <cstring>

namespace zv
{

__device__ __forceinline__ double wave_sum(double v)
{
#pragma unroll
    for (int o = 32; o > 0; o >>= 1) v += __shfl_xor(v, o, 64);
    return v;
}
__device__ __forceinline__ float wave_sum_f(float v)
{
#pragma unroll
    for (int o = 32; o > 0; o >>= 1) v += __shfl_xor(v, o, 64);
    return v;
}

typedef float floatx16m __attribute__((ext_vector_type(16)));

__global__ __launch_bounds__(256) void stats_partial_kernel(const float *__restrict__ x, int ldx, int C,
                                                            double *__restrict__ part, int nblk, const Segs segs, int rate)
{
    __shared__ double red[2][4][64];
    const int useg = blockIdx.z, blk = blockIdx.y;
    const Seg sg = seg_at(segs, useg);
    const int L = sg.rows * rate;
    if (blk * 32 >= L) return;
    const int cl = threadIdx.x & 63, rg = threadIdx.x >> 6;
    const int c = blockIdx.x * 64 + cl;
    const float *xs = x + (size_t)sg.row0 * rate * ldx;
    double s1 = 0.0, s2 = 0.0;
    if (c < C)
#pragma unroll
        for (int i = 0; i < 8; i++)
        {
            const int t = blk * 32 + rg * 8 + i;
            const double v = (t < L) ? (double)xs[(size_t)t * ldx + c] : 0.0;
            s1 += v;
            s2 += v * v;
        }
    red[0][rg][cl] = s1;
    red[1][rg][cl] = s2;
    __syncthreads();
    if (rg == 0 && c < C)
    {
        const double a = (red[0][0][cl] + red[0][1][cl]) + (red[0][2][cl] + red[0][3][cl]);
        const double b = (red[1][0][cl] + red[1][1][cl]) + (red[1][2][cl] + red[1][3][cl]);
        *(double2 *)(part + (((size_t)useg * nblk + blk) * C + c) * 2) = make_double2(a, b);
    }
}

hipError_t launch_stats_partial(hipStream_t s, const float *x, int ldx, int C, double *part, int nblk, const Segs &segs, int rate)
{
    const int nb = (segs.max_rows * rate + 31) / 32;
    if (nb > nblk || segs.nseg < 1) return hipErrorInvalidValue;
    hipLaunchKernelGGL(stats_partial_kernel, dim3((C + 63) / 64, nb, segs.nseg), dim3(256), 0, s, x, ldx, C, part, nblk, segs, rate);
    return hipGetLastError();
}

__device__ __forceinline__ float2 stats_from_partials(const double *__restrict__ p, int C, int nb, int L, float eps, int gap_at = 0, int G = 0)
{
    double s1, s2;
    dec_run_block_sum(p, (size_t)C * 2, nb, gap_at, G, &s1, &s2);
    const double mean = s1 / (double)L;
    double var = s2 / (double)L - mean * mean;
    var = var > 0.0 ? var : 0.0;
    return make_float2((float)mean, 1.0f / sqrtf((float)var + eps));
}

__device__ __forceinline__ int2 dec_run_gap(const Segs &segs, int useg, int dec_runs)
{
    if (!dec_runs || !segs.tab) return make_int2(0, 0);
    return make_int2(__builtin_amdgcn_readfirstlane(segs.tab[useg].aux), __builtin_amdgcn_readfirstlane(segs.tab[useg].pad));
}

__global__ __launch_bounds__(64) void stats_finalize_kernel(const double *__restrict__ part, int nblk, int C, float eps,
                                                            float *__restrict__ stat, int stat_seg, int c_off,
                                                            const Segs segs, int rate, int dec_runs)
{
    const int useg = blockIdx.y;
    const Seg sg = seg_at(segs, useg);
    const int L = sg.rows * rate;
    const int c = blockIdx.x * 64 + threadIdx.x;
    if (c >= C || L <= 0) return;
    const int2 gap = dec_run_gap(segs, useg, dec_runs);
    const float2 mr = stats_from_partials(part + ((size_t)useg * nblk * C + c) * 2, C, (L + 31) >> 5, L + DEC_RUN_BLOCK * gap.y, eps, gap.x, gap.y);
    float *o = stat + (size_t)useg * stat_seg + 2 * (c_off + c);
    o[0] = mr.x;
    o[1] = mr.y;
}

hipError_t launch_stats_finalize(hipStream_t s, const double *part, int nblk, int C, float eps, float *stat, int stat_seg,
                                 int c_off, const Segs &segs, int rate, int dec_runs)
{
    if (segs.nseg < 1 || (dec_runs && (!segs.tab || rate != 1))) return hipErrorInvalidValue;
    hipLaunchKernelGGL(stats_finalize_kernel, dim3((C + 63) / 64, segs.nseg), dim3(64), 0, s, part, nblk, C, eps, stat, stat_seg,
                       c_off, segs, rate, dec_runs);
    return hipGetLastError();
}

__global__ __launch_bounds__(256) void norm_apply_kernel(const float *__restrict__ x, int ldx, int C,
                                                         const float *__restrict__ stat, int stat_seg,
                                                         const float *__restrict__ g, const float *__restrict__ b,
                                                         float *__restrict__ y, int ldy, double *__restrict__ part, int nblk,
                                                         const Segs segs)
{
    __shared__ double red[2][4][64];
    const int useg = blockIdx.z, blk = blockIdx.y;
    const Seg sg = seg_at(segs, useg);
    const int L = sg.rows;
    if (blk * 32 >= L) return;
    const int cl = threadIdx.x & 63, rg = threadIdx.x >> 6;
    const int c = blockIdx.x * 64 + cl;
    const float *xs = x + (size_t)sg.row0 * ldx;
    float *ys = y + (size_t)sg.row0 * ldy;
    double s1 = 0.0, s2 = 0.0;
    if (c < C)
    {
        const float mean = stat[(size_t)useg * stat_seg + 2 * c], rstd = stat[(size_t)useg * stat_seg + 2 * c + 1];
        const float gc = g[c], bc = b[c];
#pragma unroll
        for (int i = 0; i < 8; i++)
        {
            const int t = blk * 32 + rg * 8 + i;
            if (t < L)
            {
                float v = (xs[(size_t)t * ldx + c] - mean) * rstd;
                v = v * gc;
                v = v + bc;
                ys[(size_t)t * ldy + c] = v;
                s1 += (double)v;
                s2 += (double)v * (double)v;
            }
        }
    }
    if (!part) return;
    red[0][rg][cl] = s1;
    red[1][rg][cl] = s2;
    __syncthreads();
    if (rg == 0 && c < C)
    {
        const double a = (red[0][0][cl] + red[0][1][cl]) + (red[0][2][cl] + red[0][3][cl]);
        const double q = (red[1][0][cl] + red[1][1][cl]) + (red[1][2][cl] + red[1][3][cl]);
        *(double2 *)(part + (((size_t)useg * nblk + blk) * C + c) * 2) = make_double2(a, q);
    }
}

hipError_t launch_norm_apply(hipStream_t s, const float *x, int ldx, int C, const float *stat, int stat_seg, const float *g,
                             const float *b, float *y, int ldy, double *part, int nblk, const Segs &segs)
{
    const int nb = (segs.max_rows + 31) / 32;
    if ((part && nb > nblk) || segs.nseg < 1) return hipErrorInvalidValue;
    hipLaunchKernelGGL(norm_apply_kernel, dim3((C + 63) / 64, nb, segs.nseg), dim3(256), 0, s, x, ldx, C, stat, stat_seg, g, b, y,
                       ldy, part, nblk, segs);
    return hipGetLastError();
}

__global__ __launch_bounds__(256) void norm_act_f16_kernel(const float *__restrict__ x, int ldx, int C,
                                                           const double *__restrict__ part, int nblk, int Cpart, float eps,
                                                           float *__restrict__ stat, int stat_seg,
                                                           const float *__restrict__ ga, const float *__restrict__ be, int gb_seg,
                                                           float slope, _Float16 *__restrict__ y, int ldy, _Float16 *__restrict__ yraw,
                                                           const Segs segs, int dec_runs)
{
    __shared__ float sm[4][64];
    const int useg = blockIdx.y;
    const Seg sg = seg_at(segs, useg);
    const int L = sg.rows;
    if (L <= 0) return;
    const int tid = threadIdx.x;
    if (tid < 64)
    {
        const int c = blockIdx.x * 64 + tid;
        float2 mr = make_float2(0.f, 0.f);
        float g = 0.f, b = 0.f;
        if (c < C)
        {
            float *st = stat + (size_t)useg * stat_seg + 2 * c;
            if (c < Cpart)
            {
                const int2 gap = dec_run_gap(segs, useg, dec_runs);
                mr = stats_from_partials(part + ((size_t)useg * nblk * Cpart + c) * 2, Cpart, (L + 31) >> 5, L + DEC_RUN_BLOCK * gap.y, eps, gap.x, gap.y);
                st[0] = mr.x;
                st[1] = mr.y;
            }
            else
                mr = make_float2(st[0], st[1]);
            g = ga[(size_t)useg * gb_seg + c];
            b = be[(size_t)useg * gb_seg + c];
        }
        sm[0][tid] = mr.x;
        sm[1][tid] = mr.y;
        sm[2][tid] = g;
        sm[3][tid] = b;
    }
    __syncthreads();
    const int c4 = (tid & 15) * 4, rl = tid >> 4;
    const int c = blockIdx.x * 64 + c4;
    if (c >= C) return;
    const float4 mean = *(const float4 *)&sm[0][c4], rstd = *(const float4 *)&sm[1][c4];
    const float4 g = *(const float4 *)&sm[2][c4], b = *(const float4 *)&sm[3][c4];
    const float *xs = x + (size_t)sg.row0 * ldx + c;
    _Float16 *ys = y + (size_t)sg.row0 * ldy + c;
    _Float16 *yr = yraw ? yraw + (size_t)sg.row0 * ldy + c : nullptr;
    typedef _Float16 half4v __attribute__((ext_vector_type(4)));
    for (int t0 = blockIdx.z * 128 + rl; t0 < L; t0 += 128 * gridDim.z)
    {
        float4 v[8];
#pragma unroll
        for (int u = 0; u < 8; u++)
        {
            const int t = t0 + 16 * u;
            v[u] = *(const float4 *)(xs + (size_t)(t < L ? t : L - 1) * ldx);
        }
#pragma unroll
        for (int u = 0; u < 8; u++)
        {
            const int t = t0 + 16 * u;
            if (t >= L) continue;
            float4 r;
            r.x = ((v[u].x - mean.x) * rstd.x) * g.x + b.x;
            r.y = ((v[u].y - mean.y) * rstd.y) * g.y + b.y;
            r.z = ((v[u].z - mean.z) * rstd.z) * g.z + b.z;
            r.w = ((v[u].w - mean.w) * rstd.w) * g.w + b.w;
            half4v h;
            h[0] = (_Float16)(r.x > 0.f ? r.x : r.x * slope);
            h[1] = (_Float16)(r.y > 0.f ? r.y : r.y * slope);
            h[2] = (_Float16)(r.z > 0.f ? r.z : r.z * slope);
            h[3] = (_Float16)(r.w > 0.f ? r.w : r.w * slope);
            *(half4v *)(ys + (size_t)t * ldy) = h;
            if (yr)
            {
                half4v hr;
                hr[0] = (_Float16)v[u].x;
                hr[1] = (_Float16)v[u].y;
                hr[2] = (_Float16)v[u].z;
                hr[3] = (_Float16)v[u].w;
                *(half4v *)(yr + (size_t)t * ldy) = hr;
            }
        }
    }
}

hipError_t launch_norm_act_f16(hipStream_t s, const float *x, int ldx, int C, const double *part, int nblk, int Cpart, float eps,
                               float *stat, int stat_seg, const float *ga, const float *be, int gb_seg, float slope, void *y,
                               int ldy, const Segs &segs, void *yraw, int dec_runs)
{
    if ((C & 3) || (ldx & 3) || (ldy & 3) || segs.nseg < 1 || Cpart > C || (dec_runs && !segs.tab)) return hipErrorInvalidValue;
    if (Cpart > 0 && (segs.max_rows + 31) / 32 > nblk) return hipErrorInvalidValue;
    int gz = 1;
    while (gz < 8 && (long)((C + 63) / 64) * segs.nseg * gz < 2048 && gz * 128 < segs.max_rows) gz <<= 1;
    hipLaunchKernelGGL(norm_act_f16_kernel, dim3((C + 63) / 64, segs.nseg, gz), dim3(256), 0, s, x, ldx, C, part, nblk, Cpart, eps, stat,
                       stat_seg, ga, be, gb_seg, slope, (_Float16 *)y, ldy, (_Float16 *)yraw, segs, dec_runs);
    return hipGetLastError();
}

typedef _Float16 half4v __attribute__((ext_vector_type(4)));
__global__ __launch_bounds__(256) void act_f16_kernel(const float4 *__restrict__ x0, const float4 *__restrict__ x1,
                                                      const float4 *__restrict__ x2, float pscale, float slope,
                                                      half4v *__restrict__ out, size_t n4)
{
    const size_t stride = (size_t)gridDim.x * 256;
    for (size_t i0 = (size_t)blockIdx.x * 256 + threadIdx.x; i0 < n4; i0 += 4 * stride)
    {
        float4 v[4], a[4], b[4];
#pragma unroll
        for (int u = 0; u < 4; u++)
        {
            const size_t i = i0 + u * stride;
            if (i >= n4) continue;
            v[u] = x0[i];
            if (x1)
            {
                a[u] = x1[i];
                b[u] = x2[i];
            }
        }
#pragma unroll
        for (int u = 0; u < 4; u++)
        {
            const size_t i = i0 + u * stride;
            if (i >= n4) continue;
            float4 x = v[u];
            if (x1)
            {
                x.x = ((x.x + a[u].x) + b[u].x) * pscale;
                x.y = ((x.y + a[u].y) + b[u].y) * pscale;
                x.z = ((x.z + a[u].z) + b[u].z) * pscale;
                x.w = ((x.w + a[u].w) + b[u].w) * pscale;
            }
            else
            {
                x.x = x.x * pscale;
                x.y = x.y * pscale;
                x.z = x.z * pscale;
                x.w = x.w * pscale;
            }
            half4v h;
            h[0] = (_Float16)(x.x > 0.f ? x.x : x.x * slope);
            h[1] = (_Float16)(x.y > 0.f ? x.y : x.y * slope);
            h[2] = (_Float16)(x.z > 0.f ? x.z : x.z * slope);
            h[3] = (_Float16)(x.w > 0.f ? x.w : x.w * slope);
            __builtin_nontemporal_store(h, out + i);
        }
    }
}

hipError_t launch_act_f16(hipStream_t s, const float *x0, const float *x1, const float *x2, float pscale, float slope, void *out,
                          size_t n)
{
    if ((n & 3) || !x0 || (!x1) != (!x2)) return hipErrorInvalidValue;
    const size_t n4 = n >> 2;
    const size_t wgs = std::min<size_t>((n4 + 1023) / 1024, (size_t)1 << 20);
    if (wgs == 0) return hipSuccess;
    hipLaunchKernelGGL(act_f16_kernel, dim3((unsigned)wgs), dim3(256), 0, s, (const float4 *)x0, (const float4 *)x1, (const float4 *)x2,
                       pscale, slope, (half4v *)out, n4);
    return hipGetLastError();
}

template <int RT>
__global__ __launch_bounds__(256) void linear_mfma_kernel(const float *__restrict__ x, int ldx, int in,
                                                          const float *__restrict__ W, const float *__restrict__ b, int out,
                                                          float *__restrict__ y, int ldy, const float *__restrict__ extra,
                                                          const Segs segs, int tps)
{
    __shared__ float Xs[32 * RT][33];
    __shared__ float Ws[128][33];
    const int useg = blockIdx.y / tps;
    const Seg sg = seg_at(segs, useg);
    const int n = sg.rows;
    const int n0 = (blockIdx.y - useg * tps) * 32 * RT;
    if (n0 >= n) return;
    const float *xs = x + (size_t)sg.row0 * ldx;
    float *ys = y + (size_t)sg.row0 * ldy;
    const int tid = threadIdx.x, lane = tid & 63, wave = tid >> 6;
    const int o0 = blockIdx.x * 128;
    const int i = lane & 31, kk = lane >> 5;
    floatx16m acc0, acc1;
#pragma unroll
    for (int r = 0; r < 16; r++) acc0[r] = acc1[r] = 0.f;
    float4 xv[RT], wv[4];
    auto fetch = [&](int k0) {
#pragma unroll
        for (int u = 0; u < RT; u++)
        {
            const int idx = tid + u * 256, r = idx >> 3, c = (idx & 7) * 4;
            const bool kin = k0 + c < in;
            const int row = n0 + r;
            xv[u] = (kin && row < n) ? *(const float4 *)(xs + (size_t)row * ldx + k0 + c) : make_float4(0.f, 0.f, 0.f, 0.f);
        }
#pragma unroll
        for (int u = 0; u < 4; u++)
        {
            const int idx = tid + u * 256, r = idx >> 3, c = (idx & 7) * 4;
            const bool kin = k0 + c < in;
            const int col = o0 + r;
            wv[u] = (kin && col < out) ? *(const float4 *)(W + (size_t)col * in + k0 + c) : make_float4(0.f, 0.f, 0.f, 0.f);
        }
    };
    fetch(0);
    for (int k0 = 0; k0 < in; k0 += 32)
    {
        __syncthreads();
#pragma unroll
        for (int u = 0; u < RT; u++)
        {
            const int idx = tid + u * 256, r = idx >> 3, c = (idx & 7) * 4;
            Xs[r][c] = xv[u].x; Xs[r][c + 1] = xv[u].y; Xs[r][c + 2] = xv[u].z; Xs[r][c + 3] = xv[u].w;
        }
#pragma unroll
        for (int u = 0; u < 4; u++)
        {
            const int idx = tid + u * 256, r = idx >> 3, c = (idx & 7) * 4;
            Ws[r][c] = wv[u].x; Ws[r][c + 1] = wv[u].y; Ws[r][c + 2] = wv[u].z; Ws[r][c + 3] = wv[u].w;
        }
        __syncthreads();
        if (k0 + 32 < in) fetch(k0 + 32);
#pragma unroll
        for (int k = 0; k < 32; k += 2)
        {
            const float wk = Ws[wave * 32 + i][k + kk];
            acc0 = __builtin_amdgcn_mfma_f32_32x32x2f32(Xs[i][k + kk], wk, acc0, 0, 0, 0);
            if constexpr (RT == 2) acc1 = __builtin_amdgcn_mfma_f32_32x32x2f32(Xs[32 + i][k + kk], wk, acc1, 0, 0, 0);
        }
    }
    const int col = o0 + wave * 32 + i;
    if (col >= out) return;
    const float bias = b ? b[col] : 0.f;
    const float ex = extra ? extra[col] : 0.f;
#pragma unroll
    for (int hf = 0; hf < RT; hf++)
#pragma unroll
        for (int r = 0; r < 16; r++)
        {
            const int t = n0 + hf * 32 + (r & 3) + 8 * (r >> 2) + 4 * kk;
            if (t < n)
            {
                float v = (hf ? acc1[r] : acc0[r]) + bias;
                if (extra) v = v + ex;
                ys[(size_t)t * ldy + col] = v;
            }
        }
}

hipError_t launch_linear(hipStream_t s, const float *x, int ldx, int in, const float *W, const float *b, int out, float *y,
                         int ldy, const float *extra, const Segs &segs)
{
    if ((in & 3) || (ldx & 3) || segs.nseg < 1) return hipErrorInvalidValue;
    const long wg64 = (long)((segs.max_rows + 63) / 64) * segs.nseg * ((out + 127) / 128);
    if (wg64 >= 256)
    {
        const int tps = (segs.max_rows + 63) / 64;
        hipLaunchKernelGGL(linear_mfma_kernel<2>, dim3((out + 127) / 128, tps * segs.nseg), dim3(256), 0, s, x, ldx, in, W, b, out, y,
                           ldy, extra, segs, tps);
    }
    else
    {
        const int tps = (segs.max_rows + 31) / 32;
        hipLaunchKernelGGL(linear_mfma_kernel<1>, dim3((out + 127) / 128, tps * segs.nseg), dim3(256), 0, s, x, ldx, in, W, b, out, y,
                           ldy, extra, segs, tps);
    }
    return hipGetLastError();
}

__global__ void embed_kernel(const int32_t *__restrict__ ids, const int32_t *__restrict__ puncts,
                             const float *__restrict__ wemb, int emb, const float *__restrict__ pemb, int pdim,
                             const float *__restrict__ posenc, float *__restrict__ x, int ld, const Segs segs)
{
    const Seg sg = seg_at(segs, blockIdx.y);
    const int n = blockIdx.x;
    if (n >= sg.rows) return;
    const size_t row = (size_t)sg.row0 + n;
    const int E = emb + pdim;
    const int id = ids[row], p = puncts[row];
    for (int e = threadIdx.x; e < E; e += blockDim.x)
    {
        const float v = (e < emb) ? wemb[(size_t)id * emb + e] : pemb[(size_t)p * pdim + (e - emb)];
        x[row * ld + e] = v + posenc[(size_t)n * E + e];
    }
}

hipError_t launch_embed(hipStream_t s, const int32_t *ids, const int32_t *puncts, const float *wemb, int emb,
                        const float *pemb, int pdim, const float *posenc, float *x, int ld, const Segs &segs)
{
    hipLaunchKernelGGL(embed_kernel, dim3(segs.max_rows, segs.nseg), dim3(256), 0, s, ids, puncts, wemb, emb, pemb, pdim, posenc, x,
                       ld, segs);
    return hipGetLastError();
}

template <bool VEC>
__device__ __forceinline__ void att_stage64(float *dst, int dstride, const float *src, int ld, int key0, int n, int c4n, int tid)
{
    const int total = 64 * c4n;
    for (int base = tid; base < total; base += 256 * 8)
    {
        float4 t[8];
        int off[8];
#pragma unroll
        for (int u = 0; u < 8; u++)
        {
            const int idx = base + u * 256 < total ? base + u * 256 : total - 1;
            const int r = idx / c4n, c4 = idx - r * c4n;
            const int key = key0 + r;
            t[u] = *(const float4 *)(src + (size_t)(key < n ? key : n - 1) * ld + c4 * 4);
            if (key >= n) t[u] = make_float4(0.f, 0.f, 0.f, 0.f);
            off[u] = r * dstride + c4 * 4;
        }
#pragma unroll
        for (int u = 0; u < 8; u++)
        {
            if (base + u * 256 >= total) continue;
            float *d = dst + off[u];
            if constexpr (VEC)
                *(float4 *)d = t[u];
            else
            {
                d[0] = t[u].x; d[1] = t[u].y; d[2] = t[u].z; d[3] = t[u].w;
            }
        }
    }
}

__device__ __forceinline__ float lds_read_f32(const float *p)
{
    float v;
    asm volatile("ds_read_b32 %0, %1" : "=v"(v) : "v"((unsigned)(uintptr_t)p));
    return v;
}
template <int ND, int NDMAX>
__device__ __forceinline__ void att_pv_block(floatx16m (&oacc)[NDMAX], const float *pkb, const float *Vs, int dk, int hh, int nk,
                                             const int (&doff)[NDMAX], const bool (&dok)[NDMAX])
{
    const int npb = (nk + 1) >> 1;
    float a[2][4], bv[2][4][ND];
    auto issue_pair = [&](float &ar, float (&br)[ND], int s0, int u) {
        const int kl = 2 * (s0 + u) + hh;
        const int klc = kl < nk ? kl : 0;
        ar = lds_read_f32(pkb + (size_t)klc * 64);
        const float *vr = Vs + klc * dk;
#pragma unroll
        for (int i = 0; i < ND; i++) br[i] = lds_read_f32(vr + doff[i]);
    };
    auto arrive = [&](float (&ar)[4], float (&br)[4][ND]) {
        asm volatile("s_waitcnt lgkmcnt(0)" : "+v"(ar[0]), "+v"(ar[1]), "+v"(ar[2]), "+v"(ar[3]));
#pragma unroll
        for (int u = 0; u < 4; u++)
#pragma unroll
            for (int i = 0; i < ND; i++) asm volatile("" : "+v"(br[u][i]));
// ... 720 lines not shown
        if (tid == 0)
        {
            const int total = lr_part[255];
            n_frames[blockIdx.y] = total < T ? total : T;
        }
    }
    const int f = f0 + (tid >> 4), l16 = tid & 15;
    if (f >= T) return;
    int lo = 0, hi = n;
    while (lo < hi)
    {
        const int mid = (lo + hi) >> 1;
        if (lr_cs[mid] > f) hi = mid; else lo = mid + 1;
    }
    const bool live = lo < n;
    const float4 *src = (const float4 *)(feat + ((size_t)tk.row0 + (live ? lo : 0)) * ld);
    float4 *dst = (float4 *)(hidden + ((size_t)fr.row0 + f) * ldh);
    for (int c4 = l16; c4 < (C >> 2); c4 += 16)
    {
        const float4 v = src[c4];
        dst[c4] = live ? v : make_float4(0.f, 0.f, 0.f, 0.f);
    }
}

hipError_t launch_length_regulator(hipStream_t s, const float *feat, int ld, const float *logdur, int C, float *hidden,
                                   int ldh, int32_t *cum, int32_t *n_frames, const Segs &tokens, const Segs &frames, const float *ctl,
                                   const float *pctl)
{
    if (tokens.nseg != frames.nseg || tokens.nseg < 1) return hipErrorInvalidValue;
    const bool fused_fits = tokens.max_rows >= 1 && tokens.max_rows <= 1024;
    if ((C & 3) == 0 && (ld & 3) == 0 && (ldh & 3) == 0 && fused_fits && frames.max_rows >= 1)
    {
        hipLaunchKernelGGL(lr_fused16_kernel, dim3((frames.max_rows + 15) / 16, frames.nseg), dim3(256), 0, s, feat, ld, logdur, C, hidden,
                           ldh, cum, n_frames, tokens, frames, ctl, pctl);
        return hipGetLastError();
    }
    hipLaunchKernelGGL(lr_scan_kernel, dim3(tokens.nseg), dim3(1024), 0, s, logdur, cum, n_frames, tokens, frames, ctl, pctl);
    if ((C & 3) == 0 && (ld & 3) == 0 && (ldh & 3) == 0 && (size_t)tokens.max_rows * 4 <= 48 * 1024 && tokens.max_rows >= 1)
        hipLaunchKernelGGL(lr_gather16_kernel, dim3((frames.max_rows + 15) / 16, frames.nseg), dim3(256), (size_t)tokens.max_rows * 4, s,
                           feat, ld, cum, C, hidden, ldh, tokens, frames);
    else
        hipLaunchKernelGGL(lr_gather_kernel, dim3(frames.max_rows, frames.nseg), dim3(256), 0, s, feat, ld, cum, C, hidden, ldh, tokens,
                           frames);
    return hipGetLastError();
}

__device__ __forceinline__ long long fit_block_sum(long long v, long long *red)
{
    const int tid = threadIdx.x;
    __syncthreads();
    red[tid] = v;
    __syncthreads();
    for (int o = 512; o > 0; o >>= 1)
    {
        if (tid < o) red[tid] += red[tid + o];
        __syncthreads();
    }
    return red[0];
}

__global__ __launch_bounds__(1024) void fit_durations_kernel(const float *__restrict__ logdur, const float *__restrict__ ctl,
                                                             float *__restrict__ pctl, const Segs tokens, const Segs frames)
{
    extern __shared__ long long fit_lds[];
    __shared__ long long red[1024];
    const Seg tk = seg_at(tokens, blockIdx.x), fr = seg_at(frames, blockIdx.x);
    const float *cv = ctl + (size_t)blockIdx.x * CTL_STRIDE;
    const int target = (int)cv[CTL_TARGET];
    const int n = tk.rows < tokens.max_rows ? tk.rows : tokens.max_rows, T = fr.rows;
    if (target <= 0 || n <= 0) return;
    const int nwalk = tk.aux < n ? tk.aux : n;
    const int tid = threadIdx.x;
    long long *qs = fit_lds, *rs = fit_lds + tokens.max_rows;
    float *rows = pctl + (size_t)tk.row0 * PCTL_STRIDE;
    const float *ld_ = logdur + tk.row0;
    const float dscale = cv[CTL_DURATION];
    long long Fs = 0, Q = 0, n_free = 0;
    for (int i = tid; i < nwalk; i += 1024)
    {
        const float *pr = rows + (size_t)i * PCTL_STRIDE;
        const float f = pr[PCTL_FRAMES];
        long long q = -1;
        if (f >= 0.f)
        {
            const int forced = (int)f;
            Fs += forced < T ? forced : T;
        }
        else
        {
            float dur = (float)(exp((double)ld_[i]) - 1.0);
            dur = dur * dscale;
            dur = dur * pr[PCTL_DURATION];
            q = fit_weight(dur);
            Q += q;
            n_free++;
        }
        qs[i] = q;
    }
    Fs = fit_block_sum(Fs, red);
    Q = fit_block_sum(Q, red);
    n_free = fit_block_sum(n_free, red);
    const long long R = (long long)target - Fs;
    if (R <= 0 || n_free == 0)
    {
        for (int i = tid; i < nwalk; i += 1024)
            if (qs[i] >= 0) rows[(size_t)i * PCTL_STRIDE + PCTL_FRAMES] = 0.f;
        return;
    }
    const bool equal = Q == 0;
    if (equal) Q = n_free;
    long long shares = 0;
    for (int i = tid; i < nwalk; i += 1024)
    {
        const long long q = equal ? 1 : qs[i];
        const bool is_free = qs[i] >= 0;
        const long long base = is_free ? fit_share(q, R, Q) : -1;
        rs[i] = is_free ? fit_remainder(q, R, Q) : -1;
        qs[i] = base;
        if (is_free) shares += base;
    }
    const long long L = R - fit_block_sum(shares, red);
    for (int i = tid; i < nwalk; i += 1024)
    {
        const long long ri = rs[i];
        if (ri < 0) continue;
        long long before = 0;
        if (L > 0)
            for (int j = 0; j < nwalk; j++) before += fit_before(rs[j], j, ri, i) ? 1 : 0;
        const long long d = qs[i] + (before < L ? 1 : 0);
        rows[(size_t)i * PCTL_STRIDE + PCTL_FRAMES] = (float)d;
    }
}

hipError_t launch_fit_durations(hipStream_t s, const float *logdur, const float *ctl, const float *pctl, const Segs &tokens,
                                const Segs &frames)
{
    if (!logdur || !ctl || !pctl || tokens.nseg != frames.nseg || tokens.nseg < 1 || tokens.max_rows < 1) return hipErrorInvalidValue;
    if (tokens.max_rows > FIT_MAX_TOKENS) return hipErrorInvalidValue;
    const size_t lds = (size_t)tokens.max_rows * 2 * sizeof(long long);
    hipLaunchKernelGGL(fit_durations_kernel, dim3(tokens.nseg), dim3(1024), lds, s, logdur, ctl, const_cast<float *>(pctl), tokens, frames);
    return hipGetLastError();
}

__global__ __launch_bounds__(64) void live_frames_kernel(const int32_t *__restrict__ n_frames, Seg *__restrict__ live, const Segs frames)
{
    const int u = blockIdx.x * 64 + threadIdx.x;
    if (u >= frames.nseg) return;
    const Seg cap = frames.tab ? frames.tab[u] : frames.one;
    int nf = n_frames[u];
    nf = nf < 0 ? 0 : (nf < cap.rows ? nf : cap.rows);
    *(int4 *)(live + u) = make_int4(cap.row0, nf, 0, 0);
}

hipError_t launch_live_frames(hipStream_t s, const int32_t *n_frames, Seg *live, const Segs &frames)
{
    if (frames.nseg < 1 || !n_frames || !live || (!frames.tab && frames.nseg != 1)) return hipErrorInvalidValue;
    hipLaunchKernelGGL(live_frames_kernel, dim3((frames.nseg + 63) / 64), dim3(64), 0, s, n_frames, live, frames);
    return hipGetLastError();
}

__global__ __launch_bounds__(256) void zero_tail_kernel(float *__restrict__ x, int C, const Segs frames, const Segs live, int rate)
{
    const Seg cap = seg_at(frames, blockIdx.y), lv = seg_at(live, blockIdx.y);
    const long end = (long)cap.rows * rate * C;
    long lo = (long)(lv.rows < cap.rows ? lv.rows : cap.rows) * rate * C;
    if (lo < 0) lo = 0;
    const long i0 = (long)blockIdx.x * 1024;
    if (i0 + 1024 <= lo || i0 >= end) return;
    float *xs = x + (size_t)cap.row0 * rate * C;
#pragma unroll
    for (int k = 0; k < 4; k++)
    {
        const long i = i0 + k * 256 + threadIdx.x;
        if (i >= lo && i < end) xs[i] = 0.f;
    }
}

hipError_t launch_zero_tail(hipStream_t s, float *x, int C, const Segs &frames, const Segs &live, int rate)
{
    if (frames.nseg < 1 || frames.nseg != live.nseg || frames.max_rows < 1 || C < 1 || rate < 1 || !live.tab) return hipErrorInvalidValue;
    const long per_seg = (long)frames.max_rows * rate * C;
    hipLaunchKernelGGL(zero_tail_kernel, dim3((unsigned)((per_seg + 1023) / 1024), frames.nseg), dim3(256), 0, s, x, C, frames, live, rate);
    return hipGetLastError();
}

__global__ __launch_bounds__(256) void voc_run_flags_kernel(const uint32_t *__restrict__ mel, int M, int32_t *__restrict__ eq, const Segs frames)
{
    const Seg sg = seg_at(frames, blockIdx.y);
    const int t = blockIdx.x * 4 + (threadIdx.x >> 6), lane = threadIdx.x & 63;
    if (t >= sg.rows) return;
    int same = t > 0;
    if (t > 0)
    {
        const uint32_t *r = mel + (size_t)(sg.row0 + t) * M;
        for (int c = lane; c < M; c += 64) same &= r[c] == r[c - M];
    }
    same = __all(same);
    if (lane == 0) eq[sg.row0 + t] = same;
}

__global__ __launch_bounds__(256) void voc_run_scan_kernel(const int32_t *__restrict__ eq, Seg *__restrict__ runs, const Segs frames, int H)
{
    __shared__ int s_pre[256], s_suf[256], s_len[256], s_pos[256];
    const Seg sg = seg_at(frames, blockIdx.x);
    const int T = sg.rows, tid = threadIdx.x;
    const int per = (T + 255) / 256;
    const int p0 = tid * per < T ? tid * per : T, p1 = p0 + per < T ? p0 + per : T;
    int pre = 0, cur = 0, best = 0, pos = p0;
    bool lead = true;
    for (int t = p0; t < p1; t++)
    {
        if (eq[sg.row0 + t])
        {
            cur++;
            if (lead) pre = cur;
            if (cur > best) { best = cur; pos = t - cur + 1; }
        }
        else
        {
            cur = 0;
            lead = false;
        }
    }
    s_pre[tid] = pre;
    s_suf[tid] = cur;
    s_len[tid] = best;
    s_pos[tid] = pos;
    __syncthreads();
    if (tid != 0) return;
    int run = 0, run_pos = 0, len = 0, at = 0;
    for (int k = 0; k < 256; k++)
    {
        const int q0 = k * per < T ? k * per : T, n = (q0 + per < T ? q0 + per : T) - q0;
        if (n <= 0) break;
        if (run == 0) run_pos = q0;
        if (s_pre[k] == n)
            run += n;
        else
        {
            if (run + s_pre[k] > len) { len = run + s_pre[k]; at = run_pos; }
            if (s_len[k] > len) { len = s_len[k]; at = s_pos[k]; }
            run = s_suf[k];
            run_pos = q0 + n - run;
        }
        if (run > len) { len = run; at = run_pos; }
    }
    const int a = at - 1, b = at + len, Rmin = 2 * H + 1;
    const bool take = len > 0 && b - a >= Rmin + VOC_RUN_MARGIN;
    const int shift = take ? b - a - Rmin : 0;
    *(int4 *)(runs + blockIdx.x) = make_int4(sg.row0, T - shift, take ? a + H : T, shift);
}

__global__ __launch_bounds__(256) void voc_run_compact_kernel(const uint32_t *__restrict__ mel, uint32_t *__restrict__ dst, int M, const Seg *__restrict__ runs, int H)
{
    const int4 e = *(const int4 *)(runs + blockIdx.y);
    const int row0 = __builtin_amdgcn_readfirstlane(e.x), rows = __builtin_amdgcn_readfirstlane(e.y);
    const int split = __builtin_amdgcn_readfirstlane(e.z), shift = __builtin_amdgcn_readfirstlane(e.w);
    const long n = (long)rows * M, keep = (long)(split + H + 1) * M;
    const size_t base = (size_t)row0 * M;
#pragma unroll
    for (int k = 0; k < 4; k++)
    {
        const long i = (long)blockIdx.x * 1024 + k * 256 + threadIdx.x;
        if (i < n) dst[base + i] = mel[base + i + (i >= keep ? (long)shift * M : 0)];
    }
}

hipError_t launch_voc_runs(hipStream_t s, const float *mel, int M, float *mel_c, int32_t *eq, Seg *runs, const Segs &frames, int H)
{
    if (frames.nseg < 1 || frames.max_rows < 1 || M < 1 || H < 0 || !mel || !mel_c || !eq || !runs) return hipErrorInvalidValue;
    hipLaunchKernelGGL(voc_run_flags_kernel, dim3((frames.max_rows + 3) / 4, frames.nseg), dim3(256), 0, s, (const uint32_t *)mel, M, eq, frames);
    hipLaunchKernelGGL(voc_run_scan_kernel, dim3(frames.nseg), dim3(256), 0, s, eq, runs, frames, H);
    const long per_seg = (long)frames.max_rows * M;
    hipLaunchKernelGGL(voc_run_compact_kernel, dim3((unsigned)((per_seg + 1023) / 1024), frames.nseg), dim3(256), 0, s,
                       (const uint32_t *)mel, (uint32_t *)mel_c, M, runs, H);
    return hipGetLastError();
}

__global__ __launch_bounds__(256) void voc_run_fill_kernel(float *__restrict__ x, const Seg *__restrict__ runs, int rate)
{
    const int4 e = *(const int4 *)(runs + blockIdx.y);
    const int row0 = __builtin_amdgcn_readfirstlane(e.x), split = __builtin_amdgcn_readfirstlane(e.z);
    const int shift = __builtin_amdgcn_readfirstlane(e.w);
    const long n = (long)shift * rate, i0 = (long)blockIdx.x * 1024;
    if (i0 >= n) return;
    const float *src = x + (size_t)(row0 + split) * rate;
    float *dst = x + (size_t)(row0 + split + 1) * rate;
#pragma unroll
    for (int k = 0; k < 4; k++)
    {
        const long i = i0 + k * 256 + threadIdx.x;
        if (i < n) dst[i] = src[i % rate];
    }
}

hipError_t launch_voc_run_fill(hipStream_t s, float *x, const Segs &runs, int rate)
{
    if (runs.nseg < 1 || runs.max_rows < 1 || rate < 1 || !runs.tab || !x) return hipErrorInvalidValue;
    const long per_seg = (long)runs.max_rows * rate;
    hipLaunchKernelGGL(voc_run_fill_kernel, dim3((unsigned)((per_seg + 1023) / 1024), runs.nseg), dim3(256), 0, s, x, runs.tab, rate);
    return hipGetLastError();
}

__global__ __launch_bounds__(64) void dec_runs_kernel(const int32_t *__restrict__ n_frames, Seg *__restrict__ runs, const Segs frames, int R)
{
    const int u = blockIdx.x * 64 + threadIdx.x;
    if (u >= frames.nseg) return;
    const Seg cap = frames.tab ? frames.tab[u] : frames.one;
    const DecRun r = dec_run(n_frames[u], cap.rows, R);
    *(int4 *)(runs + u) = make_int4(cap.row0, r.rows_c, r.gap_at, r.G);
}

hipError_t launch_dec_runs(hipStream_t s, const int32_t *n_frames, Seg *runs, const Segs &frames, int R)
{
    if (frames.nseg < 1 || !n_frames || !runs || R < 0 || (!frames.tab && frames.nseg != 1)) return hipErrorInvalidValue;
    hipLaunchKernelGGL(dec_runs_kernel, dim3((frames.nseg + 63) / 64), dim3(64), 0, s, n_frames, runs, frames, R);
    return hipGetLastError();
}

__global__ __launch_bounds__(256) void dec_run_expand_kernel(const float *__restrict__ src, float *__restrict__ dst, int M,
                                                             const Seg *__restrict__ runs, const Segs frames)
{
    const Seg cap = seg_at(frames, blockIdx.y);
    const int4 e = *(const int4 *)(runs + blockIdx.y);
    const int rows_c = __builtin_amdgcn_readfirstlane(e.y), gap_at = __builtin_amdgcn_readfirstlane(e.z), G = __builtin_amdgcn_readfirstlane(e.w);
    const long n = (long)cap.rows * M;
    const size_t base = (size_t)cap.row0 * M;
#pragma unroll
    for (int k = 0; k < 4; k++)
    {
        const long i = (long)blockIdx.x * 1024 + k * 256 + threadIdx.x;
        if (i >= n) continue;
        const int t = (int)(i / M), c = (int)(i - (long)t * M);
        const int tc = dec_run_compact_row(t, gap_at, G);
        if (tc < rows_c) dst[base + i] = src[base + (size_t)tc * M + c];
    }
}

hipError_t launch_dec_run_expand(hipStream_t s, const float *mel_c, float *mel, int M, const Segs &runs, const Segs &frames)
{
    if (frames.nseg < 1 || frames.nseg != runs.nseg || frames.max_rows < 1 || M < 1 || !runs.tab || !mel_c || !mel) return hipErrorInvalidValue;
    const long per_seg = (long)frames.max_rows * M;
    hipLaunchKernelGGL(dec_run_expand_kernel, dim3((unsigned)((per_seg + 1023) / 1024), frames.nseg), dim3(256), 0, s, mel_c, mel, M,
                       runs.tab, frames);
    return hipGetLastError();
}

}
```

zerovox.cpp_amd/csrc/model.h:

```cpp
#pragma once

#include <cstdint>
#include <cstring>
#include <string>
#include <vector>

#include "common.h"
#include "gguf_reader.h"
#include "kernels.h"

namespace zv
{

struct ConvW
{
    void  *w = nullptr;
    void  *w8 = nullptr;
    float *bias = nullptr;
    int    K = 0, Cin = 0, Cout = 0, Cin_p = 0, Cout_p = 0, ck = 0;
};

struct DeviceArena
{
    char  *base = nullptr;
    size_t cap = 0, used = 0;
    static size_t align(size_t off) { return (off + 255) & ~(size_t)255; }
    static DeviceArena counter() { return DeviceArena{nullptr, SIZE_MAX, 0}; }
    void  *take(size_t bytes)
    {
        const size_t a = align(used);
        if (a + bytes > cap) fail(ZV_ERR_OOM, "device arena overflow (%zu + %zu > %zu)", a, bytes, cap);
        used = a + bytes;
        return base ? base + a : nullptr;
    }
    template <typename T> T *take_n(size_t n) { return (T *)take(n * sizeof(T)); }
};

struct ProfEntry
{
    const char *name;
    hipEvent_t  e0, e1;
    double      bytes, flops;
    int         launches;
};

struct Batch
{
    int        nseg = 1;
    int        n_max = 0, t_max = 0;
    int        n_real = 0;
    size_t     n_rows = 0, t_rows = 0;
    const Seg *d_tok = nullptr, *d_frm = nullptr;
    Seg        tok1{0, 0, 0, 0}, frm1{0, 0, 0, 0};
    const float *d_ctl = nullptr;
    const float *d_pctl = nullptr;
    int32_t *d_cum = nullptr;
    Seg *d_frm_live = nullptr;
    Seg *d_dec_runs = nullptr;
    bool has_targets = false;

    static Batch single(uint32_t N, uint32_t T, uint32_t num_phonemes)
    {
        Batch b;
        b.n_max = (int)N;
        b.n_real = (int)N;
        b.t_max = (int)T;
        b.n_rows = N;
        b.t_rows = T;
        b.tok1 = Seg{0, (int32_t)N, (int32_t)num_phonemes, 0};
        b.frm1 = Seg{0, (int32_t)T, 0, 0};
        return b;
    }
    Segs tokens() const { return Segs{d_tok, nseg, n_max, tok1}; }
    Segs tokens_merged() const { return d_tok ? Segs{d_tok + nseg, 1, (int)n_rows, tok1} : tokens(); }
    Segs frames_cap() const { return Segs{d_frm, nseg, t_max, frm1}; }
    Segs frames() const { return d_frm_live ? Segs{d_frm_live, nseg, t_max, frm1} : frames_cap(); }
    bool same_schedule(const Batch &o) const
    {
        return nseg == o.nseg && n_max == o.n_max && t_max == o.t_max && n_rows == o.n_rows && t_rows == o.t_rows && d_tok == o.d_tok &&
               d_frm == o.d_frm && (d_tok || memcmp(&tok1, &o.tok1, sizeof(Seg)) == 0) && (d_frm || memcmp(&frm1, &o.frm1, sizeof(Seg)) == 0) &&
               d_ctl == o.d_ctl && d_pctl == o.d_pctl && d_cum == o.d_cum && d_frm_live == o.d_frm_live && has_targets == o.has_targets &&
               d_dec_runs == o.d_dec_runs;
    }
};

struct CapturedGraph
{
    static constexpr int NKEY = 8;
    int            kind = 0;
    unsigned       epoch = 0;
    Batch          b;
    const void    *p[NKEY] = {};
    hipGraphExec_t exec = nullptr;
    const Seg     *runs_tab = nullptr;
    int            runs_n = 0;
};

class Model
{
  public:
    Model(const std::string &gguf_path, int device);
    ~Model();

    zv_hparams hp{};
    int        device = 0;
    int        n_cu = 256;
    hipStream_t stream() const { return lanes_[cur_lane_].stream; }

    void vocode_dev(const Batch &b, const float *d_mel, float *d_wav);
    void vocode_group(const Batch &b, const float *d_mel, float *d_wav, int part = 0, int seg0 = 0);
    void vocode_tail(const Batch &b, const float *d_mel, float *d_wav, int g0, int cnt);
    hipStream_t copy_stream();
    hipEvent_t  tail_event(int i);
    static constexpr int BATCH_RING = 64;
    uint64_t    next_batch_seq() { return batch_seq_++; }
    uint64_t    batch_seq() const { return batch_seq_; }
    hipEvent_t  batch_event(uint64_t seq, int which);
    void decode_dev(const Batch &b, const float *d_hidden, const float *d_styles, float *d_mel);
    struct EncoderTaps
    {
        float   *features = nullptr, *logdur = nullptr, *pitch = nullptr, *energy = nullptr;
        int32_t *pitch_bucket = nullptr, *energy_bucket = nullptr, *cum = nullptr;
    };
    EncoderTaps encode_dev(const Batch &b, const int32_t *d_ids, const int32_t *d_puncts, const float *d_styles,
                           float *d_hidden, int32_t *d_nframes);

    struct DebugLayer
    {
        int          kind = -1, index = 0;
        const float *x = nullptr;
        float       *out = nullptr;
        bool         done = false;
    } dbg_layer;

    uint32_t max_phonemes() const { return (uint32_t)enc_.posenc_rows; }
    void reserve(uint32_t max_phonemes, uint32_t max_frames);
    void reserve_batch(const Batch &b);
    int  voc_stage_rate(int stage) const;
    int  voc_stage_channels(int stage) const;
    uint32_t max_frames_per_utterance() const;
    int wemb_rows() const { return enc_.wemb_rows; }
    int pemb_rows() const { return enc_.pemb_rows; }
    uint32_t vocoder_halo_frames() const;
    bool voc_runs_off = false;
    bool voc_runs_on(const Batch &b) const;
    const Seg *voc_runs_last(int *n) { *n = lane().runs_n; return lane().runs_tab; }
    bool dec_runs_on(const Batch &b) const;
    bool dec_prepass_on(const Batch &b) const;
    int  dec_reach_frames() const;
    void sync();

    void select_lane(int i);
    int  selected_lane() const { return cur_lane_; }
    void sync_all_lanes();
    void poison_lane(int i, int byte, size_t filled[3]);

    void *io_scratch(size_t bytes);
    void *pinned_scratch(size_t bytes);

    bool graph_mode = false;
    void vocode_dev_graph(const Batch &b, const float *d_mel, float *d_wav);
    void chain_dev(const Batch &b, const int32_t *d_ids, const int32_t *d_puncts, const float *d_styles, float *d_hidden,
                   float *d_mel, float *d_wav, int32_t *d_nframes, const void *h2d_src = nullptr, void *h2d_dst = nullptr,
                   size_t h2d_bytes = 0, int voc_part = 0);

    bool profiling = false;
    std::vector<ProfEntry> prof;
    void prof_clear();

    uint32_t E() const { return hp.emb_dim + hp.punct_emb_dim; }
    void debug_layernorm(int index, uint32_t n);

  private:
    std::vector<void *> allocs_;
    void  *dev_alloc(size_t bytes);
    float *upload_f32(const GgufTensor &t, int pad_to = 0, float pad_value = 0.f);
    float *upload_vec(const GgufFile &g, const std::string &name, int expect_n, int pad_to = 0, float pad_value = 0.f);
    ConvW  load_conv(const GgufFile &g, const std::string &wname, const std::string &bname, int expect_cin = -1, bool gemm_pack = false);
    ConvW  load_upsample(const GgufFile &g, int idx, int stride, int expect_cin);

    struct ResPair { ConvW c1, c2; void *p1 = nullptr, *p2 = nullptr, *r1 = nullptr, *r2 = nullptr, *x1 = nullptr, *x2 = nullptr; };
    struct Voc
    {
        float *mean = nullptr, *scale = nullptr;
        ConvW  in_conv;
        int    n_up = 0;
        int    scales[8] = {0};
        ConvW  ups[8];
        int    n_rb = 0, n_dil = 3;
        int    dil[8] = {1, 3, 5};
        std::vector<ResPair> pairs;
        uint16_t *out_w = nullptr;
        float  out_b = 0.f;
        int    out_K = 0, out_C = 0;
    } voc_;
    VocGeom voc_geom_{};
    VocCall voc_call(const Batch &b) const;
    TripleJob block_job(const ResPair *rp, int n_dil, bool ring, const float *y, float *out) const;
    struct DilPairJobs { ConvJob c1, c2; PairJob p; };
    DilPairJobs pair_jobs(const ResPair &rp, int dil, const float *yin, float *yout, _Float16 *xt, float *y) const;

    struct DecBlk
    {
        ConvW  conv1, conv2, sc;
        bool   learned_sc = false;
        int    cin = 0, cout = 0;
        float *n1w = nullptr, *n1b = nullptr, *n2w = nullptr, *n2b = nullptr;
        int    g1 = 0, g2 = 0;
    };
    struct Dec
    {
        DecBlk enc[2], dec[5];
        ConvW  asr0, to_out;
        float *asr1w = nullptr, *asr1b = nullptr;
        float *fcW = nullptr, *fcB = nullptr, *fcExtra = nullptr;
        int    fc_out = 0;
        int    R = 64, M = 80;
    } dec_;

    struct EncLayer
    {
        float *qkvW = nullptr, *qkvB = nullptr, *fcW = nullptr, *fcB = nullptr;
        float *ln1w = nullptr, *ln1b = nullptr, *ln2w = nullptr, *ln2b = nullptr;
        ConvW  w1, w2;
    };
    struct VarPred
    {
        ConvW  c1, c2;
        float *l1w = nullptr, *l1b = nullptr, *l2w = nullptr, *l2b = nullptr, *lw = nullptr, *lb = nullptr;
        int    V = 0;
    };
    struct Enc
    {
        float *wemb = nullptr, *pemb = nullptr, *posenc = nullptr, *pitch_emb = nullptr, *energy_emb = nullptr;
        int    posenc_rows = 0, wemb_rows = 0, pemb_rows = 0;
        std::vector<EncLayer> layers;
        VarPred dur, pitch, energy;
    } enc_;

    struct VocLayout
    {
        float *c0;
        struct Stage { float *ub, *y[3]; _Float16 *xt[3]; } st[8];
        float *mel_c; int32_t *eq; Seg *runs;
    };
    struct DecLayout
    {
        int    nblk, hs, ss;
        float *h, *st_x, *st_t, *st_y, *st_a, *cat, *t1, *sc, *x0, *xa, *asr_t;
        double *part_t, *part_o; _Float16 *xa16, *t16, *xr16;
        float *mel_c;
    };
    struct EncLayout { int Vp; float *x, *y, *qkv, *o, *f, *va, *vb; _Float16 *hh; EncoderTaps t; };
    VocLayout voc_layout(DeviceArena &a, const Batch &b) const;
    DecLayout dec_layout(DeviceArena &a, const Batch &b) const;
    EncLayout enc_layout(DeviceArena &a, const Batch &b) const;
    static constexpr size_t ARENA_TAIL = (size_t)1 << 20;
    size_t arena_bytes_for(const Batch &b) const;
    void  arena_require(size_t bytes);
    DeviceArena &stage_arena(const Batch &b);

    void conv(const ConvJob *jobs, int n, const Segs &segs, int rate, const char *name, double bytes, double flops);
    void dbg_inject(void *dev, int ld, int cols, size_t rows);
    void dbg_extract(const void *dev, int ld, int cols, size_t rows);
    ConvJob job(const ConvW &w) const;
    void tick(hipEvent_t *e0);
    void tock(hipEvent_t e0, const char *name, double bytes, double flops);
    void group_begin();
    void group_end(const char *name);
    bool       in_group_ = false;
    hipEvent_t group_e0_ = nullptr;
    double     group_bytes_ = 0.0, group_flops_ = 0.0;
    int        group_n_ = 0;

    struct Lane
    {
        hipStream_t stream = nullptr;
        DeviceArena arena;
        void       *io = nullptr;
        size_t      io_cap = 0;
        void       *pinned = nullptr;
        size_t      pinned_cap = 0;
        hipStream_t copy_stream = nullptr;
        std::vector<hipEvent_t> tail_events;
        const Seg  *runs_tab = nullptr;
        int         runs_n = 0;
    };
    std::vector<Lane> lanes_;
    int  cur_lane_ = 0;
    Lane &lane() { return lanes_[cur_lane_]; }
    uint64_t   batch_seq_ = 0;
    hipEvent_t batch_events_[2 * BATCH_RING] = {};

    bool skip_launch_ = false;
    std::vector<CapturedGraph> graphs_;
    void drop_graphs();
    template <typename F> void run_captured(int kind, const Batch &b, const void *const (&key)[CapturedGraph::NKEY], F &&enqueue);
};

}
```

Before: 33460.

## Pack decoder run rows contiguously so convs run as one dense segment

When the decoder uses compacted run tables in a batch, each utterance's live rows are packed back-to-back into 32-row slots, and the decoder convs run over a single packed segment instead of per-utterance padded segments. A prefix-scan kernel assigns packed offsets, a pack kernel copies the hidden rows, and the stats, normalisation and expand kernels are taught the packed block indexing plus tail handling for partial blocks. This aims to cut padding work and improve tile occupancy in batched decoder convs, at the cost of an extra copy pass and more complex stats bookkeeping.

```diff
diff --git a/zerovox.cpp_amd/csrc/capi.cpp b/zerovox.cpp_amd/csrc/capi.cpp
--- a/zerovox.cpp_amd/csrc/capi.cpp
+++ b/zerovox.cpp_amd/csrc/capi.cpp
@@ -613,7 +613,7 @@
     const size_t o_nf = dev.at((size_t)bt.nseg * 4), o_in = dev.at(b_in), o_hid = dev.at(bt.t_rows * E * 4),
                  o_mel = dev.at(bt.t_rows * Mm * 4), o_wav = dev.at(bt.t_rows * hop * 4), o_cum = dev.at(dur ? bt.n_rows * 4 : 0),
                  o_live = dev.at(r.fitted ? (size_t)bt.nseg * sizeof(zv::Seg) : 0),
-                 o_runs = dev.at(!r.fitted ? (size_t)bt.nseg * sizeof(zv::Seg) : 0);
+                 o_runs = dev.at(!r.fitted ? (size_t)(bt.nseg + 1) * sizeof(zv::Seg) : 0);
     M.reserve_batch(bt);
     char *io = (char *)M.io_scratch(dev.size());
     size_t wav_bytes = 0;
diff --git a/zerovox.cpp_amd/csrc/conv_plan.h b/zerovox.cpp_amd/csrc/conv_plan.h
--- a/zerovox.cpp_amd/csrc/conv_plan.h
+++ b/zerovox.cpp_amd/csrc/conv_plan.h
@@ -19,10 +19,26 @@
 
 inline int plan_round_up(int x, int a) { return (x + a - 1) / a * a; }
 
+inline int &conv_packed_utts()
+{
+    static thread_local int n = 0;
+    return n;
+}
+struct ConvPackedUtts
+{
+    int saved;
+    explicit ConvPackedUtts(int n) : saved(conv_packed_utts()) { conv_packed_utts() = n; }
+    ~ConvPackedUtts() { conv_packed_utts() = saved; }
+    ConvPackedUtts(const ConvPackedUtts &) = delete;
+    ConvPackedUtts &operator=(const ConvPackedUtts &) = delete;
+};
+
 struct ConvCall
 {
     int njobs, nseg, max_rows, rate, n_cu, nt_begin;
-};
+    int nutt = conv_packed_utts();
+};
+inline bool conv_call_is_batch(const ConvCall &c) { return c.nseg > 1 || c.nutt > 1; }
 
 inline int conv_gemm_groups(int Cout_p) { return ((Cout_p + 31) / 32) / 8; }
 inline int conv_gemm_tiles(int Cout_p)
@@ -126,7 +142,7 @@
     {
         p.xcd_ny = p.gy;
         p.xcd_nx = p.gx;
-        p.xcd_spread = c.nseg > 1;
+        p.xcd_spread = conv_call_is_batch(c);
         p.gx = conv_xcd_grid(p.xcd_nx, p.xcd_ny, p.xcd_spread), p.gy = 1;
     }
     p.tile_bytes = plan_round_up((BM + halo + dmax) * (ck * 2 + 16), 16);
@@ -191,7 +207,7 @@
     if (nt_env == 1 || (nt_env == 2 && WN == 4 && ntiles >= 2 && MT >= 2)) NT = nt_env;
     if (NT == 2 && MT == 4) MT = 2;
     {
-        const bool batch_rounds = ZV_CONV_BATCH_ROUTE && c.nseg > 1 && wgs(1, 1) > n_cu;
+        const bool batch_rounds = ZV_CONV_BATCH_ROUTE && conv_call_is_batch(c) && wgs(1, 1) > n_cu;
         const int  single_env = knob(ZV_CONV_SINGLE);
         if (single_env != 0 && MT == 1 && NT == 1 && ck == 256 && wgs(1, 1) <= 2L * n_cu && !batch_rounds && (jobs[0].Cin_p > 256 || single_env == 2) &&
             WN >= 2 && conv_plan_tiles(p, true, 1, WN, 1, Lmax, ntiles, halo, ck, dmax, c))
diff --git a/zerovox.cpp_amd/csrc/dec_runs.h b/zerovox.cpp_amd/csrc/dec_runs.h
--- a/zerovox.cpp_amd/csrc/dec_runs.h
+++ b/zerovox.cpp_amd/csrc/dec_runs.h
@@ -75,4 +75,23 @@
     *sumsq = s2;
 }
 
+constexpr int DEC_PACK_SLOT = 32;
+ZV_DR_FN int dec_pack_slot(int rows_c) { return rows_c <= 0 ? 0 : (rows_c + DEC_PACK_SLOT) / DEC_PACK_SLOT * DEC_PACK_SLOT; }
+ZV_DR_FN long dec_pack_rows_cap(long t_rows, int nseg) { return t_rows + (long)DEC_PACK_SLOT * nseg; }
+
+ZV_DR_FN void dec_pack_tail_pair(const float *x, size_t ld, int rows, double *sum, double *sumsq)
+{
+    double s1[2] = {0.0, 0.0}, s2[2] = {0.0, 0.0};
+    for (int h = 0; h < 2; h++)
+        for (int r = 0; r < 16; r++)
+        {
+            const int t = 4 * h + (r & 3) + 8 * (r >> 2);
+            const double v = t < rows ? (double)x[(size_t)t * ld] : 0.0;
+            s1[h] += v;
+            s2[h] += v * v;
+        }
+    *sum = s1[0] + s1[1];
+    *sumsq = s2[0] + s2[1];
 }
+
+}
diff --git a/zerovox.cpp_amd/csrc/decoder.cpp b/zerovox.cpp_amd/csrc/decoder.cpp
--- a/zerovox.cpp_amd/csrc/decoder.cpp
+++ b/zerovox.cpp_amd/csrc/decoder.cpp
@@ -1,4 +1,5 @@
 #include "schedule.h"
+#include "dec_runs.h"
 
 #include <algorithm>
 #include <cmath>
@@ -8,11 +9,13 @@
 
 Model::DecLayout Model::dec_layout(DeviceArena &a, const Batch &bt) const
 {
-    const size_t S = (size_t)bt.nseg, L = bt.t_rows, B = 2 * E(), R = (size_t)dec_.R, CAT = B + R;
+    const size_t S = (size_t)bt.nseg, L = (size_t)dec_pack_rows_cap((long)bt.t_rows, bt.nseg), B = 2 * E(), R = (size_t)dec_.R, CAT = B + R;
     DecLayout d{(bt.t_max + 31) / 32, round_up(dec_.fc_out + 64, 64), 2 * (int)CAT + 64};
+    d.rows = (int)L;
+    d.nblk_all = std::max(bt.nseg * d.nblk, (d.rows + 31) / 32);
     d.h = a.take_n<float>(S * d.hs);
     for (float **st : {&d.st_x, &d.st_t, &d.st_y, &d.st_a}) *st = a.take_n<float>(S * d.ss);
-    for (double **p : {&d.part_t, &d.part_o}) *p = a.take_n<double>(S * d.nblk * CAT * 2);
+    for (double **p : {&d.part_t, &d.part_o}) *p = a.take_n<double>((size_t)d.nblk_all * CAT * 2);
     d.cat = a.take_n<float>(L * CAT);
     for (float **x : {&d.t1, &d.sc, &d.x0, &d.xa}) *x = a.take_n<float>(L * B);
     d.asr_t = a.take_n<float>(L * R);
@@ -35,6 +38,8 @@
     return !bt.d_frm_live && dbg_layer.kind < 0 && dec_prepass_on(bt) && batch_switch(k, batch_rows((long)bt.t_rows));
 }
 
+bool Model::dec_pack_on(const Batch &bt) const { return bt.d_dec_runs != nullptr && bt.nseg > 1 && knob(ZV_DEC_PACK) != 0; }
+
 int Model::dec_reach_frames() const
 {
     auto half = [](const ConvW &w) { return w.K > 0 ? (w.K - 1) / 2 : 0; };
@@ -51,6 +56,11 @@
     const bool runs = bt.d_dec_runs != nullptr;
     if (runs && !dec_runs_on(bt)) fail(ZV_ERR_ARG, "internal: a decoder run table on a schedule that takes none");
     const Segs fr = runs ? Segs{bt.d_dec_runs, bt.nseg, bt.t_max, bt.frm1} : bt.frames();
+    const bool pack = runs && dec_pack_on(bt);
+    const Segs frc = pack ? Segs{bt.d_dec_runs + bt.nseg, 1, lay.rows, Seg{0, 0, 0, 0}} : fr;
+    const ConvPackedUtts packed_utts(pack ? bt.nseg : 0);
+    const int tab_mode = runs ? DEC_TAB_RUNS | (pack ? DEC_TAB_PACKED : 0) : 0, conv_tail = pack ? DEC_TAB_CONV_TAIL : 0;
+    const int nblk_c = pack ? lay.nblk_all : lay.nblk;
     const int Ed = (int)E(), B = 2 * Ed, R = dec_.R, CAT = B + R, S = bt.nseg;
     const size_t L = bt.t_rows;
     const int nblk = lay.nblk, hs = lay.hs, ss = lay.ss;
@@ -74,16 +84,17 @@
 
     const float rsqrt2 = (float)(1.0 / sqrt(2.0));
 
-    auto finalize = [&](const double *part, int C, float *stat, int c_off) {
+    auto finalize = [&](const double *part, int C, float *stat, int c_off, const float *xconv = nullptr, int ldxc = 0) {
         ZV_LAUNCH("dec_in_stats", 16.0 * S * nblk * C, 4.0 * S * nblk * C,
-                  launch_stats_finalize(stream(), part, nblk, C, 1e-5f, stat, ss, c_off, fr, 1, runs));
+                  launch_stats_finalize(stream(), part, nblk, C, 1e-5f, stat, ss, c_off, fr, 1, tab_mode | (xconv ? conv_tail : 0), xconv, ldxc));
     };
     auto norm_input = [&](ConvJob &j, const float *x, int ldx, int C, const double *part, int Cpart, float *stat, const float *g,
-                          const float *b, int gb_seg, _Float16 *op16, _Float16 *raw16 = nullptr) {
+                          const float *b, int gb_seg, bool from_conv, _Float16 *op16, _Float16 *raw16 = nullptr) {
         if (prepass)
         {
             ZV_LAUNCH("dec_norm_operand", 6.0 * Ld * C, 8.0 * Ld * C,
-                      launch_norm_act_f16(stream(), x, ldx, C, part, nblk, Cpart, 1e-5f, stat, ss, g, b, gb_seg, 0.2f, op16, C, fr, raw16, runs));
+                      launch_norm_act_f16(stream(), x, ldx, C, part, nblk, Cpart, 1e-5f, stat, ss, g, b, gb_seg, 0.2f, op16, C, fr, raw16,
+                                          tab_mode | (from_conv ? conv_tail : 0)));
             j.x0 = op16;
             j.ldx = C;
             j.pro = PRO_RAW_F16;
@@ -103,10 +114,16 @@
         }
     };
 
-    ZV_LAUNCH("dec_in_stats", 4.0 * Ld * Ed, 3.0 * Ld * Ed, launch_stats_partial(stream(), d_hidden, Ed, Ed, part_o, nblk, fr, 1));
+    const float *hidden = d_hidden;
+    if (pack)
+    {
+        ZV_LAUNCH("dec_pack_rows", 8.0 * Ld * Ed, 0.0, launch_dec_pack_rows(stream(), d_hidden, xa, Ed, fr, bt.frames_cap()));
+        hidden = xa;
+    }
+    ZV_LAUNCH("dec_in_stats", 4.0 * Ld * Ed, 3.0 * Ld * Ed, launch_stats_partial(stream(), hidden, Ed, Ed, part_o, nblk, fr, 1, pack));
 
     int blk_no = 0;
-    auto block = [&](const DecBlk &b, const float *x, int ldx, int Cpart, float *st_in, const float *g1, const float *b1,
+    auto block = [&](const DecBlk &b, const float *x, int ldx, int Cpart, bool x_from_conv, float *st_in, const float *g1, const float *b1,
                      const float *g2, const float *b2, int gb_seg, float *out, int ldo, bool want_stats) {
         const bool dbg_here = dbg_layer.kind == 2 && dbg_layer.index == blk_no && !dbg_layer.done;
         blk_no++;
@@ -116,6 +133,7 @@
             dbg_inject(const_cast<float *>(x), ldx, b.cin, L);
             ZV_HIP(launch_stats_partial(stream(), x, ldx, b.cin, part_o, nblk, fr, 1));
             Cpart = b.cin;
+            x_from_conv = false;
         }
         const float *res = x;
         int ldres = ldx;
@@ -123,10 +141,10 @@
         int nj = 0;
         {
             ConvJob j = job(b.conv1);
-            norm_input(j, x, ldx, b.cin, part_o, Cpart, st_in, g1, b1, gb_seg, xa16, b.learned_sc ? xr16 : nullptr);
+            norm_input(j, x, ldx, b.cin, part_o, Cpart, st_in, g1, b1, gb_seg, x_from_conv, xa16, b.learned_sc ? xr16 : nullptr);
             j.out = t1;
             j.stat_part = part_t;
-            j.stat_nblk = nblk;
+            j.stat_nblk = nblk_c;
             j.stat_C = b.conv1.Cout;
             jj[nj++] = j;
         }
@@ -153,13 +171,13 @@
                 flops += sf;
             }
             else
-                conv(&j, 1, fr, 1, "dec_conv", sb, sf);
-        }
-        conv(jj, nj, fr, 1, "dec_conv", bytes, flops);
+                conv(&j, 1, frc, 1, "dec_conv", sb, sf);
+        }
+        conv(jj, nj, frc, 1, "dec_conv", bytes, flops);
         const int Cm = b.conv1.Cout;
         {
             ConvJob j = job(b.conv2);
-            norm_input(j, t1, b.conv1.Cout_p, Cm, part_t, Cm, st_t, g2, b2, gb_seg, t16);
+            norm_input(j, t1, b.conv1.Cout_p, Cm, part_t, Cm, st_t, g2, b2, gb_seg, true, t16);
             j.res = res;
             j.ldres = ldres;
             j.escale = rsqrt2;
@@ -168,10 +186,10 @@
             if (want_stats)
             {
                 j.stat_part = part_o;
-                j.stat_nblk = nblk;
+                j.stat_nblk = nblk_c;
                 j.stat_C = b.cout;
             }
-            conv(&j, 1, fr, 1, "dec_conv", conv_bytes(Ld, Cm, b.cout, 3, true), conv_flops(Ld, Cm, b.cout, 3));
+            conv(&j, 1, frc, 1, "dec_conv", conv_bytes(Ld, Cm, b.cout, 3, true), conv_flops(Ld, Cm, b.cout, 3));
         }
         if (dbg_here) dbg_extract(out, ldo, b.cout, L);
     };
@@ -191,22 +209,22 @@
         return;
     }
 
-    block(dec_.enc[0], d_hidden, Ed, Ed, st_x, dec_.enc[0].n1w, dec_.enc[0].n1b, dec_.enc[0].n2w, dec_.enc[0].n2b, 0, x0, B, true);
-    block(dec_.enc[1], x0, B, B, st_y, dec_.enc[1].n1w, dec_.enc[1].n1b, dec_.enc[1].n2w, dec_.enc[1].n2b, 0, cat, CAT, true);
+    block(dec_.enc[0], hidden, Ed, Ed, false, st_x, dec_.enc[0].n1w, dec_.enc[0].n1b, dec_.enc[0].n2w, dec_.enc[0].n2b, 0, x0, B, true);
+    block(dec_.enc[1], x0, B, B, true, st_y, dec_.enc[1].n1w, dec_.enc[1].n1b, dec_.enc[1].n2w, dec_.enc[1].n2b, 0, cat, CAT, true);
 
     if (dbg_layer.done) return;
     {
         ConvJob j = job(dec_.asr0);
-        j.x0 = d_hidden;
+        j.x0 = hidden;
         j.ldx = Ed;
         j.out = asr_t;
         j.stat_part = part_t;
-        j.stat_nblk = nblk;
+        j.stat_nblk = nblk_c;
         j.stat_C = R;
-        conv(&j, 1, fr, 1, "dec_conv", conv_bytes(Ld, Ed, R, 1, false), conv_flops(Ld, Ed, R, 1));
-        finalize(part_t, R, st_a, 0);
+        conv(&j, 1, frc, 1, "dec_conv", conv_bytes(Ld, Ed, R, 1, false), conv_flops(Ld, Ed, R, 1));
+        finalize(part_t, R, st_a, 0, asr_t, R);
         ZV_LAUNCH("dec_norm_apply", 8.0 * Ld * R, 3.0 * Ld * R,
-                  launch_norm_apply(stream(), asr_t, R, R, st_a, ss, dec_.asr1w, dec_.asr1b, cat + B, CAT, part_t, nblk, fr));
+                  launch_norm_apply(stream(), asr_t, R, R, st_a, ss, dec_.asr1w, dec_.asr1b, cat + B, CAT, part_t, nblk, fr, pack));
         finalize(part_t, R, st_x, B);
         if (dbg_layer.kind == ZV_LAYER_DEC_ASR_RES)
         {
@@ -224,7 +242,7 @@
     for (int i = 0; i < 5; i++)
     {
         const DecBlk &b = dec_.dec[i];
-        block(b, cur, ldc, cparts[i], sts[i], h + b.g1, h + b.g1 + b.cin, h + b.g2, h + b.g2 + b.cout, hs, outs[i], ldos[i], i < 4);
+        block(b, cur, ldc, cparts[i], true, sts[i], h + b.g1, h + b.g1 + b.cin, h + b.g2, h + b.g2 + b.cout, hs, outs[i], ldos[i], i < 4);
         cur = outs[i];
         ldc = ldos[i];
     }
@@ -236,7 +254,7 @@
         j.out = runs ? lay.mel_c : d_mel;
         j.ldo = dec_.M;
         if (dbg_layer.kind == ZV_LAYER_DEC_TO_OUT) dbg_inject(const_cast<float *>(cur), ldc, Ed, L);
-        conv(&j, 1, fr, 1, "dec_conv", conv_bytes(Ld, Ed, dec_.M, 1, false), conv_flops(Ld, Ed, dec_.M, 1));
+        conv(&j, 1, frc, 1, "dec_conv", conv_bytes(Ld, Ed, dec_.M, 1, false), conv_flops(Ld, Ed, dec_.M, 1));
         if (dbg_layer.kind == ZV_LAYER_DEC_TO_OUT) dbg_extract(d_mel, dec_.M, dec_.M, L);
     }
     if (runs)
diff --git a/zerovox.cpp_amd/csrc/encoder.cpp b/zerovox.cpp_amd/csrc/encoder.cpp
--- a/zerovox.cpp_amd/csrc/encoder.cpp
+++ b/zerovox.cpp_amd/csrc/encoder.cpp
@@ -152,7 +152,7 @@
     if (bt.d_frm_live)
         ZV_LAUNCH("enc_live_frames", 36.0 * bt.nseg, 0.0, launch_live_frames(stream(), d_nframes, bt.d_frm_live, fr));
     if (bt.d_dec_runs)
-        ZV_LAUNCH("enc_dec_runs", 36.0 * bt.nseg, 0.0, launch_dec_runs(stream(), d_nframes, bt.d_dec_runs, fr, dec_reach_frames()));
+        ZV_LAUNCH("enc_dec_runs", 36.0 * bt.nseg, 0.0, launch_dec_runs(stream(), d_nframes, bt.d_dec_runs, fr, dec_reach_frames(), dec_pack_on(bt)));
     return t;
 }
 
diff --git a/zerovox.cpp_amd/csrc/kernels.h b/zerovox.cpp_amd/csrc/kernels.h
--- a/zerovox.cpp_amd/csrc/kernels.h
+++ b/zerovox.cpp_amd/csrc/kernels.h
@@ -184,11 +184,13 @@
 };
 hipError_t launch_out_conv(hipStream_t s, const OutConvArgs &a);
 
-hipError_t launch_stats_partial(hipStream_t s, const float *x, int ldx, int C, double *part, int nblk, const Segs &segs, int rate);
+hipError_t launch_stats_partial(hipStream_t s, const float *x, int ldx, int C, double *part, int nblk, const Segs &segs, int rate,
+                                int packed = 0);
+constexpr int DEC_TAB_RUNS = 1, DEC_TAB_PACKED = 2, DEC_TAB_CONV_TAIL = 4;
 hipError_t launch_stats_finalize(hipStream_t s, const double *part, int nblk, int C, float eps, float *stat, int stat_seg,
-                                 int c_off, const Segs &segs, int rate, int dec_runs = 0);
+                                 int c_off, const Segs &segs, int rate, int dec_runs = 0, const float *x = nullptr, int ldx = 0);
 hipError_t launch_norm_apply(hipStream_t s, const float *x, int ldx, int C, const float *stat, int stat_seg, const float *g,
-                             const float *b, float *y, int ldy, double *part, int nblk, const Segs &segs);
+                             const float *b, float *y, int ldy, double *part, int nblk, const Segs &segs, int packed = 0);
 
 hipError_t launch_act_f16(hipStream_t s, const float *x0, const float *x1, const float *x2, float pscale, float slope, void *out, size_t n);
 hipError_t launch_norm_act_f16(hipStream_t s, const float *x, int ldx, int C, const double *part, int nblk, int Cpart, float eps,
@@ -241,7 +243,8 @@
 hipError_t launch_voc_runs(hipStream_t s, const float *mel, int M, float *mel_c, int32_t *eq, Seg *runs, const Segs &frames, int H);
 hipError_t launch_voc_run_fill(hipStream_t s, float *x, const Segs &runs, int rate);
 
-hipError_t launch_dec_runs(hipStream_t s, const int32_t *n_frames, Seg *runs, const Segs &frames, int R);
+hipError_t launch_dec_runs(hipStream_t s, const int32_t *n_frames, Seg *runs, const Segs &frames, int R, int packed = 0);
+hipError_t launch_dec_pack_rows(hipStream_t s, const float *x, float *xp, int C, const Segs &runs, const Segs &frames);
 hipError_t launch_dec_run_expand(hipStream_t s, const float *mel_c, float *mel, int M, const Segs &runs, const Segs &frames);
 
 }
diff --git a/zerovox.cpp_amd/csrc/knobs.h b/zerovox.cpp_amd/csrc/knobs.h
--- a/zerovox.cpp_amd/csrc/knobs.h
+++ b/zerovox.cpp_amd/csrc/knobs.h
@@ -21,7 +21,8 @@
     X(ZV_CONV_STREAM, 1)        \
     X(ZV_VOC_RUNS, 1)           \
     X(ZV_DEC_RUNS, 1)           \
-    X(ZV_UP_GEMM, 1)            \
+    X(ZV_DEC_PACK, 1)           \
+    X(ZV_UP_GEMM, 1)           \
     X(ZV_GEMM_ORDER, 2)         \
     X(ZV_PAIR_MT, 0)                                                                  \
     X(ZV_CONV_XCD, 1)           \
diff --git a/zerovox.cpp_amd/csrc/misc_kernels.hip b/zerovox.cpp_amd/csrc/misc_kernels.hip
--- a/zerovox.cpp_amd/csrc/misc_kernels.hip
+++ b/zerovox.cpp_amd/csrc/misc_kernels.hip
@@ -23,14 +23,20 @@
 
 typedef float floatx16m __attribute__((ext_vector_type(16)));
 
+__device__ __forceinline__ size_t part_block0(const Seg &sg, int useg, int nblk, int packed)
+{
+    return packed ? (size_t)(sg.row0 / DEC_RUN_BLOCK) : (size_t)useg * nblk;
+}
+
 __global__ __launch_bounds__(256) void stats_partial_kernel(const float *__restrict__ x, int ldx, int C,
-                                                            double *__restrict__ part, int nblk, const Segs segs, int rate)
+                                                            double *__restrict__ part, int nblk, const Segs segs, int rate, int packed)
 {
     __shared__ double red[2][4][64];
     const int useg = blockIdx.z, blk = blockIdx.y;
     const Seg sg = seg_at(segs, useg);
     const int L = sg.rows * rate;
     if (blk * 32 >= L) return;
+    const size_t blk0 = part_block0(sg, useg, nblk, packed);
     const int cl = threadIdx.x & 63, rg = threadIdx.x >> 6;
     const int c = blockIdx.x * 64 + cl;
     const float *xs = x + (size_t)sg.row0 * rate * ldx;
@@ -51,22 +57,32 @@
     {
         const double a = (red[0][0][cl] + red[0][1][cl]) + (red[0][2][cl] + red[0][3][cl]);
         const double b = (red[1][0][cl] + red[1][1][cl]) + (red[1][2][cl] + red[1][3][cl]);
-        *(double2 *)(part + (((size_t)useg * nblk + blk) * C + c) * 2) = make_double2(a, b);
-    }
-}
-
-hipError_t launch_stats_partial(hipStream_t s, const float *x, int ldx, int C, double *part, int nblk, const Segs &segs, int rate)
+        *(double2 *)(part + ((blk0 + blk) * C + c) * 2) = make_double2(a, b);
+    }
+}
+
+hipError_t launch_stats_partial(hipStream_t s, const float *x, int ldx, int C, double *part, int nblk, const Segs &segs, int rate, int packed)
 {
     const int nb = (segs.max_rows * rate + 31) / 32;
-    if (nb > nblk || segs.nseg < 1) return hipErrorInvalidValue;
-    hipLaunchKernelGGL(stats_partial_kernel, dim3((C + 63) / 64, nb, segs.nseg), dim3(256), 0, s, x, ldx, C, part, nblk, segs, rate);
-    return hipGetLastError();
-}
-
-__device__ __forceinline__ float2 stats_from_partials(const double *__restrict__ p, int C, int nb, int L, float eps, int gap_at = 0, int G = 0)
+    if (nb > nblk || segs.nseg < 1 || (packed && (!segs.tab || rate != 1))) return hipErrorInvalidValue;
+    hipLaunchKernelGGL(stats_partial_kernel, dim3((C + 63) / 64, nb, segs.nseg), dim3(256), 0, s, x, ldx, C, part, nblk, segs, rate, packed);
+    return hipGetLastError();
+}
+
+__device__ __forceinline__ float2 stats_from_partials(const double *__restrict__ p, int C, int nb, int L, float eps, int gap_at = 0, int G = 0,
+                                                      const float *__restrict__ xtail = nullptr, size_t ldx = 0, int tail = 0)
 {
     double s1, s2;
-    dec_run_block_sum(p, (size_t)C * 2, nb, gap_at, G, &s1, &s2);
+    if (xtail && tail > 0)
+    {
+        double t1, t2;
+        dec_run_block_sum(p, (size_t)C * 2, nb - 1, gap_at, G, &s1, &s2);
+        dec_pack_tail_pair(xtail, ldx, tail, &t1, &t2);
+        s1 += t1;
+        s2 += t2;
+    }
+    else
+        dec_run_block_sum(p, (size_t)C * 2, nb, gap_at, G, &s1, &s2);
     const double mean = s1 / (double)L;
     double var = s2 / (double)L - mean * mean;
     var = var > 0.0 ? var : 0.0;
@@ -75,13 +91,13 @@
 
 __device__ __forceinline__ int2 dec_run_gap(const Segs &segs, int useg, int dec_runs)
 {
-    if (!dec_runs || !segs.tab) return make_int2(0, 0);
+    if (!(dec_runs & DEC_TAB_RUNS) || !segs.tab) return make_int2(0, 0);
     return make_int2(__builtin_amdgcn_readfirstlane(segs.tab[useg].aux), __builtin_amdgcn_readfirstlane(segs.tab[useg].pad));
 }
 
 __global__ __launch_bounds__(64) void stats_finalize_kernel(const double *__restrict__ part, int nblk, int C, float eps,
                                                             float *__restrict__ stat, int stat_seg, int c_off,
-                                                            const Segs segs, int rate, int dec_runs)
+                                                            const Segs segs, int rate, int dec_runs, const float *__restrict__ x, int ldx)
 {
     const int useg = blockIdx.y;
     const Seg sg = seg_at(segs, useg);
@@ -89,18 +105,22 @@
     const int c = blockIdx.x * 64 + threadIdx.x;
     if (c >= C || L <= 0) return;
     const int2 gap = dec_run_gap(segs, useg, dec_runs);
-    const float2 mr = stats_from_partials(part + ((size_t)useg * nblk * C + c) * 2, C, (L + 31) >> 5, L + DEC_RUN_BLOCK * gap.y, eps, gap.x, gap.y);
+    const bool tail = (dec_runs & DEC_TAB_CONV_TAIL) && (L & 31);
+    const float2 mr = stats_from_partials(part + (part_block0(sg, useg, nblk, dec_runs & DEC_TAB_PACKED) * C + c) * 2, C, (L + 31) >> 5,
+                                          L + DEC_RUN_BLOCK * gap.y, eps, gap.x, gap.y,
+                                          tail ? x + ((size_t)sg.row0 + (L & ~31)) * ldx + c : nullptr, (size_t)ldx, L & 31);
     float *o = stat + (size_t)useg * stat_seg + 2 * (c_off + c);
     o[0] = mr.x;
     o[1] = mr.y;
 }
 
 hipError_t launch_stats_finalize(hipStream_t s, const double *part, int nblk, int C, float eps, float *stat, int stat_seg,
-                                 int c_off, const Segs &segs, int rate, int dec_runs)
+                                 int c_off, const Segs &segs, int rate, int dec_runs, const float *x, int ldx)
 {
     if (segs.nseg < 1 || (dec_runs && (!segs.tab || rate != 1))) return hipErrorInvalidValue;
+    if ((dec_runs & DEC_TAB_CONV_TAIL) && (!(dec_runs & DEC_TAB_PACKED) || !x)) return hipErrorInvalidValue;
     hipLaunchKernelGGL(stats_finalize_kernel, dim3((C + 63) / 64, segs.nseg), dim3(64), 0, s, part, nblk, C, eps, stat, stat_seg,
-                       c_off, segs, rate, dec_runs);
+                       c_off, segs, rate, dec_runs, x, ldx);
     return hipGetLastError();
 }
 
@@ -108,7 +128,7 @@
                                                          const float *__restrict__ stat, int stat_seg,
                                                          const float *__restrict__ g, const float *__restrict__ b,
                                                          float *__restrict__ y, int ldy, double *__restrict__ part, int nblk,
-                                                         const Segs segs)
+                                                         const Segs segs, int packed)
 {
     __shared__ double red[2][4][64];
     const int useg = blockIdx.z, blk = blockIdx.y;
@@ -147,17 +167,17 @@
     {
         const double a = (red[0][0][cl] + red[0][1][cl]) + (red[0][2][cl] + red[0][3][cl]);
         const double q = (red[1][0][cl] + red[1][1][cl]) + (red[1][2][cl] + red[1][3][cl]);
-        *(double2 *)(part + (((size_t)useg * nblk + blk) * C + c) * 2) = make_double2(a, q);
+        *(double2 *)(part + ((part_block0(sg, useg, nblk, packed) + blk) * C + c) * 2) = make_double2(a, q);
     }
 }
 
 hipError_t launch_norm_apply(hipStream_t s, const float *x, int ldx, int C, const float *stat, int stat_seg, const float *g,
-                             const float *b, float *y, int ldy, double *part, int nblk, const Segs &segs)
+                             const float *b, float *y, int ldy, double *part, int nblk, const Segs &segs, int packed)
 {
     const int nb = (segs.max_rows + 31) / 32;
-    if ((part && nb > nblk) || segs.nseg < 1) return hipErrorInvalidValue;
+    if ((part && nb > nblk) || segs.nseg < 1 || (packed && !segs.tab)) return hipErrorInvalidValue;
     hipLaunchKernelGGL(norm_apply_kernel, dim3((C + 63) / 64, nb, segs.nseg), dim3(256), 0, s, x, ldx, C, stat, stat_seg, g, b, y,
-                       ldy, part, nblk, segs);
+                       ldy, part, nblk, segs, packed);
     return hipGetLastError();
 }
 
@@ -185,7 +205,10 @@
             if (c < Cpart)
             {
                 const int2 gap = dec_run_gap(segs, useg, dec_runs);
-                mr = stats_from_partials(part + ((size_t)useg * nblk * Cpart + c) * 2, Cpart, (L + 31) >> 5, L + DEC_RUN_BLOCK * gap.y, eps, gap.x, gap.y);
+                const bool tail = (dec_runs & DEC_TAB_CONV_TAIL) && (L & 31);
+                mr = stats_from_partials(part + (part_block0(sg, useg, nblk, dec_runs & DEC_TAB_PACKED) * Cpart + c) * 2, Cpart, (L + 31) >> 5,
+                                         L + DEC_RUN_BLOCK * gap.y, eps, gap.x, gap.y,
+                                         tail ? x + ((size_t)sg.row0 + (L & ~31)) * ldx + c : nullptr, (size_t)ldx, L & 31);
                 st[0] = mr.x;
                 st[1] = mr.y;
             }
@@ -209,6 +232,15 @@
     _Float16 *ys = y + (size_t)sg.row0 * ldy + c;
     _Float16 *yr = yraw ? yraw + (size_t)sg.row0 * ldy + c : nullptr;
     typedef _Float16 half4v __attribute__((ext_vector_type(4)));
+    if ((dec_runs & DEC_TAB_PACKED) && blockIdx.z == 0)
+    {
+        const half4v z = {0, 0, 0, 0};
+        for (int t = L + rl; t < dec_pack_slot(L); t += 16)
+        {
+            *(half4v *)(ys + (size_t)t * ldy) = z;
+            if (yr) *(half4v *)(yr + (size_t)t * ldy) = z;
+        }
+    }
     for (int t0 = blockIdx.z * 128 + rl; t0 < L; t0 += 128 * gridDim.z)
     {
         float4 v[8];
@@ -1535,19 +1567,62 @@
     return hipGetLastError();
 }
 
-__global__ __launch_bounds__(64) void dec_runs_kernel(const int32_t *__restrict__ n_frames, Seg *__restrict__ runs, const Segs frames, int R)
-{
-    const int u = blockIdx.x * 64 + threadIdx.x;
-    if (u >= frames.nseg) return;
-    const Seg cap = frames.tab ? frames.tab[u] : frames.one;
-    const DecRun r = dec_run(n_frames[u], cap.rows, R);
-    *(int4 *)(runs + u) = make_int4(cap.row0, r.rows_c, r.gap_at, r.G);
-}
-
-hipError_t launch_dec_runs(hipStream_t s, const int32_t *n_frames, Seg *runs, const Segs &frames, int R)
+__global__ __launch_bounds__(64) void dec_runs_kernel(const int32_t *__restrict__ n_frames, Seg *__restrict__ runs, const Segs frames, int R,
+                                                      int packed)
+{
+    const int lane = threadIdx.x;
+    int done = 0;
+    for (int u0 = 0; u0 < frames.nseg; u0 += 64)
+    {
+        const int u = u0 + lane;
+        const bool live = u < frames.nseg;
+        const Seg cap = frames.tab ? frames.tab[live ? u : 0] : frames.one;
+        const DecRun r = dec_run(live ? n_frames[u] : 0, cap.rows, R);
+        const int slot = live && packed ? dec_pack_slot(r.rows_c) : 0;
+        int incl = slot;
+#pragma unroll
+        for (int o = 1; o < 64; o <<= 1)
+        {
+            const int v = __shfl_up(incl, o, 64);
+            if (lane >= o) incl += v;
+        }
+        if (live) *(int4 *)(runs + u) = make_int4(packed ? done + incl - slot : cap.row0, r.rows_c, r.gap_at, r.G);
+        done += __shfl(incl, 63, 64);
+    }
+    if (packed && lane == 0) *(int4 *)(runs + frames.nseg) = make_int4(0, done, 0, 0);
+}
+
+hipError_t launch_dec_runs(hipStream_t s, const int32_t *n_frames, Seg *runs, const Segs &frames, int R, int packed)
 {
     if (frames.nseg < 1 || !n_frames || !runs || R < 0 || (!frames.tab && frames.nseg != 1)) return hipErrorInvalidValue;
-    hipLaunchKernelGGL(dec_runs_kernel, dim3((frames.nseg + 63) / 64), dim3(64), 0, s, n_frames, runs, frames, R);
+    hipLaunchKernelGGL(dec_runs_kernel, dim3(1), dim3(64), 0, s, n_frames, runs, frames, R, packed);
+    return hipGetLastError();
+}
+
+__global__ __launch_bounds__(256) void dec_pack_rows_kernel(const float4 *__restrict__ src, float4 *__restrict__ dst, int C4,
+                                                            const Seg *__restrict__ runs, const Segs frames)
+{
+    const Seg cap = seg_at(frames, blockIdx.y);
+    const int4 e = *(const int4 *)(runs + blockIdx.y);
+    const int row0_p = __builtin_amdgcn_readfirstlane(e.x), rows_c = __builtin_amdgcn_readfirstlane(e.y);
+    const long n = (long)dec_pack_slot(rows_c) * C4, live = (long)rows_c * C4;
+    const float4 *sp = src + (size_t)cap.row0 * C4;
+    float4 *dp = dst + (size_t)row0_p * C4;
+#pragma unroll
+    for (int k = 0; k < 4; k++)
+    {
+        const long i = (long)blockIdx.x * 1024 + k * 256 + threadIdx.x;
+        if (i >= n) continue;
+        dp[i] = i < live ? sp[i] : make_float4(0.f, 0.f, 0.f, 0.f);
+    }
+}
+
+hipError_t launch_dec_pack_rows(hipStream_t s, const float *x, float *xp, int C, const Segs &runs, const Segs &frames)
+{
+    if (frames.nseg < 1 || frames.nseg != runs.nseg || frames.max_rows < 1 || C < 4 || (C & 3) || !runs.tab || !x || !xp) return hipErrorInvalidValue;
+    const long per_slot = (long)dec_pack_slot(frames.max_rows) * (C / 4);
+    hipLaunchKernelGGL(dec_pack_rows_kernel, dim3((unsigned)((per_slot + 1023) / 1024), frames.nseg), dim3(256), 0, s, (const float4 *)x,
+                       (float4 *)xp, C / 4, runs.tab, frames);
     return hipGetLastError();
 }
 
@@ -1558,7 +1633,7 @@
     const int4 e = *(const int4 *)(runs + blockIdx.y);
     const int rows_c = __builtin_amdgcn_readfirstlane(e.y), gap_at = __builtin_amdgcn_readfirstlane(e.z), G = __builtin_amdgcn_readfirstlane(e.w);
     const long n = (long)cap.rows * M;
-    const size_t base = (size_t)cap.row0 * M;
+    const size_t base = (size_t)cap.row0 * M, cbase = (size_t)__builtin_amdgcn_readfirstlane(e.x) * M;
 #pragma unroll
     for (int k = 0; k < 4; k++)
     {
@@ -1566,7 +1641,7 @@
         if (i >= n) continue;
         const int t = (int)(i / M), c = (int)(i - (long)t * M);
         const int tc = dec_run_compact_row(t, gap_at, G);
-        if (tc < rows_c) dst[base + i] = src[base + (size_t)tc * M + c];
+        if (tc < rows_c) dst[base + i] = src[cbase + (size_t)tc * M + c];
     }
 }
 
diff --git a/zerovox.cpp_amd/csrc/model.h b/zerovox.cpp_amd/csrc/model.h
--- a/zerovox.cpp_amd/csrc/model.h
+++ b/zerovox.cpp_amd/csrc/model.h
@@ -146,6 +146,7 @@
     bool voc_runs_on(const Batch &b) const;
     const Seg *voc_runs_last(int *n) { *n = lane().runs_n; return lane().runs_tab; }
     bool dec_runs_on(const Batch &b) const;
+    bool dec_pack_on(const Batch &b) const;
     bool dec_prepass_on(const Batch &b) const;
     int  dec_reach_frames() const;
     void sync();
@@ -247,6 +248,7 @@
     struct DecLayout
     {
         int    nblk, hs, ss;
+        int    rows, nblk_all;
         float *h, *st_x, *st_t, *st_y, *st_a, *cat, *t1, *sc, *x0, *xa, *asr_t;
         double *part_t, *part_o; _Float16 *xa16, *t16, *xr16;
         float *mel_c;
```

New measurement: 34370 (median of 6 runs). +2.7%, better.
